# HuiyangYu/TGSFilter

Measured on NVIDIA B200. Metric: filtered Gbases/s, higher is better.
Workload: dtype u8/u64

## Files before the change

include/tgsf.h:

```cpp
#ifndef TGSF_H_
#define TGSF_H_

#include <stddef.h>
#include <stdint.h>

#ifdef __cplusplus
extern "C" {
#endif

#define TGSF_OK 0
#define TGSF_ERR_INVALID 1
#define TGSF_ERR_CUDA 2
#define TGSF_ERR_NOMEM 3
#define TGSF_ERR_STATE 4
#define TGSF_ERR_CAPACITY 5

#define TGSF_DROPINFO_N 17
#define TGSF_QUAL_HIST_N 256
#define TGSF_MAX_ADAPTERS 65536
#define TGSF_MAX_ADAPTER_LEN 2048
#define TGSF_LIB_ADAPTERS 22

#define TGSF_FLAG_FILTER 1u
#define TGSF_FLAG_ONLY_QC 2u
#define TGSF_FLAG_DISCARD_MID 4u
#define TGSF_FLAG_GZ_BLOCKS 8u
#define TGSF_FLAG_GZ_FASTA 16u

typedef struct tgsf_params {
    int32_t min_len;
    int32_t max_len;
    float min_q;
    float max_q;
    int32_t bc_len;
    int32_t head_trim;
    int32_t tail_trim;
    int32_t end_len;
    int32_t end_match_len;
    int32_t mid_match_len;
    int32_t extra_len;
    float end_sim;
    float mid_sim;
    int32_t kmer;
    int32_t min_repeat;
    int32_t qtype;
    uint32_t flags;
    int32_t n_adapters;
    const uint8_t *const *adapter_seq;
    const int32_t *adapter_len;
    int32_t max_read_len;
    int32_t n_slots;
} tgsf_params;

typedef struct tgsf_read_result {
    uint64_t sum_q;
    int32_t status;
    int32_t n_mid;
    int32_t n_5p;
    int32_t n_3p;
    int32_t piece_begin;
    int32_t n_pieces;
} tgsf_read_result;

#define TGSF_READ_EVALUATED 0
#define TGSF_READ_LOWQ 1
#define TGSF_READ_EMPTY 2

typedef struct tgsf_piece {
    uint64_t sum_q;
    int32_t read;
    int32_t start;
    int32_t len;
    int32_t repeat_len;
    int32_t status;
    int32_t contam_hits;
} tgsf_piece;

#define TGSF_PIECE_EMIT 0
#define TGSF_PIECE_SHORT_REPEAT 1
#define TGSF_PIECE_LOWQ 2
#define TGSF_PIECE_QC_ONLY 3
#define TGSF_PIECE_CONTAM 4

typedef struct tgsf_counter_layout {
    uint32_t n_u64;
    uint32_t bc_len;
    uint32_t max_bins;
    uint32_t drop_info;
    uint32_t raw_hist;
    uint32_t clean_hist;
    uint32_t raw5p_cnt;
    uint32_t raw5p_qual;
    uint32_t raw3p_cnt;
    uint32_t raw3p_qual;
    uint32_t clean5p_cnt;
    uint32_t clean5p_qual;
    uint32_t clean3p_cnt;
    uint32_t clean3p_qual;
    uint32_t raw_bin_cnt;
    uint32_t raw_bin_qual;
    uint32_t clean_bin_cnt;
    uint32_t clean_bin_qual;
} tgsf_counter_layout;

typedef struct tgsf_ctx tgsf_ctx;

const char *tgsf_version(void);
const char *tgsf_last_error(void);

int tgsf_create(int device, const tgsf_params *params, tgsf_ctx **out);
int tgsf_destroy(tgsf_ctx *ctx);

int tgsf_device_count(int *count);

int tgsf_host_alloc(void **ptr, size_t bytes);
int tgsf_host_free(void *ptr);

int tgsf_submit(tgsf_ctx *ctx, const uint8_t *bases, const uint8_t *quals, const uint64_t *offsets,
                uint32_t n_reads);
int tgsf_submit_packed(tgsf_ctx *ctx, const uint8_t *packed_bases, const uint8_t *quals, const uint64_t *offsets,
                       uint32_t n_reads, const uint64_t *exc_pos, const uint8_t *exc_byte, uint64_t n_exc);
int tgsf_pack_bases(const uint8_t *bases, uint64_t n, uint8_t *packed, uint64_t *exc_pos, uint8_t *exc_byte,
                    uint64_t exc_cap, uint64_t *n_exc);
int tgsf_submit_device(tgsf_ctx *ctx, const uint8_t *d_bases, const uint8_t *d_quals,
                       const uint64_t *d_offsets, uint32_t n_reads, uint64_t n_bases);
typedef struct tgsf_gz_span {
    uint64_t offset;
    uint32_t bytes;
    uint32_t reserved;
} tgsf_gz_span;
int tgsf_collect_gz(tgsf_ctx *ctx, uint8_t *blob, uint64_t blob_cap, uint64_t *blob_bytes, tgsf_gz_span *spans,
                    uint32_t spans_cap, uint32_t *n_spans);
int tgsf_collect(tgsf_ctx *ctx, tgsf_read_result *reads, uint32_t n_reads, tgsf_piece *pieces,
                 uint32_t pieces_cap, uint32_t *n_pieces);
int tgsf_set_contaminants(tgsf_ctx *ctx, const uint8_t *seq, const uint64_t *offsets, uint32_t n_seqs, int32_t k,
                          float min_frac, uint64_t *n_kmers);

int tgsf_last_timing(tgsf_ctx *ctx, float *kernel_ms, float *total_ms);

#define TGSF_N_STAGES 7
#define TGSF_STAGE_RAW_SCAN 0
#define TGSF_STAGE_RAW_FINAL 1
#define TGSF_STAGE_MID_SCAN 2
#define TGSF_STAGE_RESOLVE 3
#define TGSF_STAGE_REGIONS 4
#define TGSF_STAGE_KMER 5
#define TGSF_STAGE_CLEAN 6
int tgsf_last_stage_ms(tgsf_ctx *ctx, float *out, int n);

int tgsf_last_span(tgsf_ctx *ctx, float *start_ms, float *end_ms);

int tgsf_counter_layout_get(const tgsf_ctx *ctx, tgsf_counter_layout *out);
int tgsf_counters(tgsf_ctx *ctx, uint64_t *out, uint32_t n_u64);
int tgsf_counters_reset(tgsf_ctx *ctx);
int tgsf_counters_device(tgsf_ctx *ctx, void **d_ptr, uint32_t *n_u64);
int tgsf_allreduce(tgsf_ctx **ctxs, int n);
uint64_t tgsf_launch_count(const tgsf_ctx *ctx);
int tgsf_launch_shape(const tgsf_ctx *ctx, int32_t *sm_count, int32_t *last_chunk_shift);

int tgsf_prepass(int device, const uint8_t *ends5p, const uint8_t *ends3p, uint32_t n,
                 uint32_t row_len, const uint8_t *const *lib_seq, const int32_t *lib_len,
                 int32_t n_lib, float min_sim, int32_t *bases_num5p, int32_t *bases_num3p,
                 int64_t *map5p, int64_t *map3p);

typedef struct tgsf_align_result {
    int32_t edit_distance;
    int32_t n_locations;
    int32_t align_len;
    int32_t first_start, first_end, last_start, last_end;
    uint32_t loc_hash;
} tgsf_align_result;
int tgsf_align_hw(int device, const uint8_t *queries, const uint32_t *q_off, const uint8_t *targets,
                  const uint32_t *t_off, const int32_t *k, uint32_t n, tgsf_align_result *out);

#ifdef __cplusplus
}
#endif
#endif
```

tgsfilter_b200/_capi.py:

```python
from __future__ import annotations

import ctypes as C
import os

_HERE = os.path.dirname(os.path.abspath(__file__))
LIB_PATH = os.environ.get("TGSF_LIB_PATH") or os.path.join(_HERE, "libtgsf_cuda.so")

TGSF_OK = 0
TGSF_ERR_INVALID = 1
TGSF_ERR_CUDA = 2
TGSF_ERR_NOMEM = 3
TGSF_ERR_STATE = 4
TGSF_ERR_CAPACITY = 5

FLAG_FILTER = 1
FLAG_ONLY_QC = 2
FLAG_DISCARD_MID = 4
FLAG_GZ_BLOCKS = 8
FLAG_GZ_FASTA = 16

READ_EVALUATED, READ_LOWQ, READ_EMPTY = 0, 1, 2
PIECE_EMIT, PIECE_SHORT_REPEAT, PIECE_LOWQ, PIECE_QC_ONLY, PIECE_CONTAM = 0, 1, 2, 3, 4

N_STAGES = 7
STAGE_NAMES = ("raw_scan", "raw_final", "mid_scan", "resolve", "regions", "kmer", "clean")
DROPINFO_N = 17
QUAL_HIST_N = 256


class Params(C.Structure):

    _fields_ = [
        ("min_len", C.c_int32),
        ("max_len", C.c_int32),
        ("min_q", C.c_float),
        ("max_q", C.c_float),
        ("bc_len", C.c_int32),
        ("head_trim", C.c_int32),
        ("tail_trim", C.c_int32),
        ("end_len", C.c_int32),
        ("end_match_len", C.c_int32),
        ("mid_match_len", C.c_int32),
        ("extra_len", C.c_int32),
        ("end_sim", C.c_float),
        ("mid_sim", C.c_float),
        ("kmer", C.c_int32),
        ("min_repeat", C.c_int32),
        ("qtype", C.c_int32),
        ("flags", C.c_uint32),
        ("n_adapters", C.c_int32),
        ("adapter_seq", C.POINTER(C.c_char_p)),
        ("adapter_len", C.POINTER(C.c_int32)),
        ("max_read_len", C.c_int32),
        ("n_slots", C.c_int32),
    ]


class ReadResult(C.Structure):
    _fields_ = [
        ("sum_q", C.c_uint64),
        ("status", C.c_int32),
        ("n_mid", C.c_int32),
        ("n_5p", C.c_int32),
        ("n_3p", C.c_int32),
        ("piece_begin", C.c_int32),
        ("n_pieces", C.c_int32),
    ]


class Piece(C.Structure):
    _fields_ = [
        ("sum_q", C.c_uint64),
        ("read", C.c_int32),
        ("start", C.c_int32),
        ("len", C.c_int32),
        ("repeat_len", C.c_int32),
        ("status", C.c_int32),
        ("contam_hits", C.c_int32),
    ]


class CounterLayout(C.Structure):
    _fields_ = [(n, C.c_uint32) for n in (
        "n_u64", "bc_len", "max_bins", "drop_info", "raw_hist", "clean_hist",
        "raw5p_cnt", "raw5p_qual", "raw3p_cnt", "raw3p_qual",
        "clean5p_cnt", "clean5p_qual", "clean3p_cnt", "clean3p_qual",
        "raw_bin_cnt", "raw_bin_qual", "clean_bin_cnt", "clean_bin_qual")]


class AlignResult(C.Structure):
    _fields_ = [(n, C.c_int32) for n in (
        "edit_distance", "n_locations", "align_len",
        "first_start", "first_end", "last_start", "last_end")] + [("loc_hash", C.c_uint32)]


READ_RESULT_DTYPE = [("sum_q", "<u8"), ("status", "<i4"), ("n_mid", "<i4"), ("n_5p", "<i4"),
                     ("n_3p", "<i4"), ("piece_begin", "<i4"), ("n_pieces", "<i4")]
PIECE_DTYPE = [("sum_q", "<u8"), ("read", "<i4"), ("start", "<i4"), ("len", "<i4"),
               ("repeat_len", "<i4"), ("status", "<i4"), ("contam_hits", "<i4")]
ALIGN_RESULT_DTYPE = [("edit_distance", "<i4"), ("n_locations", "<i4"), ("align_len", "<i4"),
                      ("first_start", "<i4"), ("first_end", "<i4"), ("last_start", "<i4"),
                      ("last_end", "<i4"), ("loc_hash", "<u4")]

EXPORTED_SYMBOLS = (
    "tgsf_version", "tgsf_last_error", "tgsf_create", "tgsf_destroy", "tgsf_device_count", "tgsf_host_alloc",
    "tgsf_host_free", "tgsf_submit", "tgsf_submit_packed", "tgsf_pack_bases", "tgsf_submit_device", "tgsf_collect", "tgsf_collect_gz", "tgsf_last_timing", "tgsf_last_span", "tgsf_last_stage_ms",
    "tgsf_counter_layout_get", "tgsf_counters", "tgsf_counters_reset", "tgsf_counters_device",
    "tgsf_launch_count", "tgsf_launch_shape", "tgsf_allreduce", "tgsf_prepass", "tgsf_align_hw", "tgsf_set_contaminants",
)

_lib = None


def load() -> C.CDLL:
    global _lib
    if _lib is not None:
        return _lib
    if not os.path.exists(LIB_PATH):
        raise RuntimeError(
            f"{LIB_PATH} is missing: build it with __graft_entry__.build() "
            "(nvcc, sm_100a). tgsfilter_b200 has no CPU fallback.")
    lib = C.CDLL(LIB_PATH)
    vp, u8p, u64p = C.c_void_p, C.c_void_p, C.c_void_p
    lib.tgsf_version.restype = C.c_char_p
    lib.tgsf_version.argtypes = []
    lib.tgsf_last_error.restype = C.c_char_p
    lib.tgsf_last_error.argtypes = []
    lib.tgsf_create.argtypes = [C.c_int, C.POINTER(Params), C.POINTER(vp)]
    lib.tgsf_destroy.argtypes = [vp]
    lib.tgsf_device_count.argtypes = [C.POINTER(C.c_int)]
    lib.tgsf_host_alloc.argtypes = [C.POINTER(vp), C.c_size_t]
    lib.tgsf_host_free.argtypes = [vp]
    lib.tgsf_submit.argtypes = [vp, u8p, u8p, u64p, C.c_uint32]
    lib.tgsf_submit_packed.argtypes = [vp, u8p, u8p, u64p, C.c_uint32, u64p, u8p, C.c_uint64]
    lib.tgsf_pack_bases.argtypes = [u8p, C.c_uint64, u8p, u64p, u8p, C.c_uint64, C.POINTER(C.c_uint64)]
    lib.tgsf_submit_device.argtypes = [vp, u8p, u8p, u64p, C.c_uint32, C.c_uint64]
    lib.tgsf_collect.argtypes = [vp, vp, C.c_uint32, vp, C.c_uint32, C.POINTER(C.c_uint32)]
    lib.tgsf_collect_gz.argtypes = [vp, vp, C.c_uint64, C.POINTER(C.c_uint64), vp, C.c_uint32, C.POINTER(C.c_uint32)]
    lib.tgsf_last_timing.argtypes = [vp, C.POINTER(C.c_float), C.POINTER(C.c_float)]
    lib.tgsf_last_span.argtypes = [vp, C.POINTER(C.c_float), C.POINTER(C.c_float)]
    lib.tgsf_last_stage_ms.argtypes = [vp, C.POINTER(C.c_float), C.c_int]
    lib.tgsf_counter_layout_get.argtypes = [vp, C.POINTER(CounterLayout)]
    lib.tgsf_counters.argtypes = [vp, u64p, C.c_uint32]
    lib.tgsf_counters_reset.argtypes = [vp]
    lib.tgsf_counters_device.argtypes = [vp, C.POINTER(vp), C.POINTER(C.c_uint32)]
    lib.tgsf_launch_count.restype = C.c_uint64
    lib.tgsf_launch_count.argtypes = [vp]
    lib.tgsf_launch_shape.argtypes = [vp, C.POINTER(C.c_int32), C.POINTER(C.c_int32)]
    lib.tgsf_allreduce.argtypes = [C.POINTER(vp), C.c_int]
    lib.tgsf_prepass.argtypes = [C.c_int, u8p, u8p, C.c_uint32, C.c_uint32,
                                 C.POINTER(C.c_char_p), C.POINTER(C.c_int32), C.c_int32, C.c_float,
                                 vp, vp, vp, vp]
    lib.tgsf_align_hw.argtypes = [C.c_int, u8p, vp, u8p, vp, vp, C.c_uint32, vp]
    lib.tgsf_set_contaminants.argtypes = [vp, u8p, u64p, C.c_uint32, C.c_int32, C.c_float, C.POINTER(C.c_uint64)]
    for name in EXPORTED_SYMBOLS:
        fn = getattr(lib, name)
        if fn.restype is C.c_int and name not in ("tgsf_version", "tgsf_last_error",
                                                   "tgsf_launch_count"):
            fn.restype = C.c_int
    _lib = lib
    return lib


class TgsfError(RuntimeError):
    def __init__(self, code: int, where: str):
        msg = ""
        try:
            msg = load().tgsf_last_error().decode("utf-8", "replace")
        except Exception:
            pass
        super().__init__(f"{where} failed with status {code}: {msg}")
        self.code = code


def check(code: int, where: str) -> None:
    if code != TGSF_OK:
        raise TgsfError(code, where)
```

tgsfilter_b200/csrc/adapters.cuh:

```cuda
#pragma once
#include "common.cuh"
#include "myers.cuh"

#define MID_THREADS 128
#define RES_THREADS 128

struct AdapterCtx {
    const DevAdapter *ad;
    const u64 *peq_pool;
};

static __device__ __forceinline__ AdapterTables adapter_tables(const AdapterCtx &C, int a) {
    const DevAdapter A = C.ad[a];
    AdapterTables T;
    T.hw = C.peq_pool + A.peq_off;
    T.fw = T.hw + 256 * A.nw;
    T.rv = T.fw + 256 * A.nw;
    T.qlen = A.qlen;
    return T;
}

struct MidScanArgs {
    int a[2];
    int end_len;
    int chunk_shift;
    u32 chunk_stride;
    int n_adapters;
};

template <int NW>
static __device__ void mid_chunk_record(const u64 *__restrict__ tab, int tab_stride, int qlen,
                                        const uint8_t *__restrict__ bases, u64 sb, u64 ob, u64 oe,
                                        int d, u32 &cnt, u64 &first) {
    Myers<NW> s;
    myers_init_hw<NW>(s, qlen);
    cnt = 0;
    first = 0;
    for (u64 p = sb; p < oe; ++p) {
        myers_step<NW, 0, true>(s, tab + (u32)bases[p] * tab_stride, 0);
        if (p >= ob && s.score == d) {
            if (cnt == 0) first = p;
            ++cnt;
        }
    }
}

template <int NW>
static __device__ __noinline__ int mid_replay_group(const u64 *P0, const u64 *M0, u32 w0, u32 w1,
                                                    const u64 *tab, int tab_stride, int best) {
    u64 tP[NW], tM[NW];
#pragma unroll
    for (int w = 0; w < NW; ++w) { tP[w] = P0[w]; tM[w] = M0[w]; }
    const u32 wd[2] = {w0, w1};
#pragma unroll 1
    for (int j = 0; j < 8; ++j) {
        const u32 byte = (wd[j >> 2] >> (8 * (j & 3))) & 0xffu;
        myers_step_state<NW>(tP, tM, tab + byte * tab_stride);
        best = min(best, myers_score<NW>(tP, tM));
    }
    return best;
}

template <int NW, int AP>
__global__ void __launch_bounds__(MID_THREADS, (NW * AP <= 2) ? 6 : 3)
k_mid_scan_dyn(DevBatch B, AdapterCtx C, MidScanArgs M, const ChunkEntry *__restrict__ chunks,
               const u32 *__restrict__ perm, const u32 *__restrict__ n_chunks_ptr,
               uint8_t *__restrict__ chunk_min,
               u32 *__restrict__ chunk_cnt, u64 *__restrict__ chunk_first,
               u32 *__restrict__ best_mid, u32 *__restrict__ work_ctr) {
    const u32 n_chunks = *n_chunks_ptr;
    extern __shared__ __align__(16) u64 s_peq_smem[];
    DevAdapter A[AP];
#pragma unroll
    for (int x = 0; x < AP; ++x) A[x] = C.ad[M.a[x]];
    const u64 *s_peq = s_peq_smem;
    if (NW > 4) {
        s_peq = C.peq_pool + A[0].peq_off;
    } else {
#pragma unroll
        for (int x = 0; x < AP; ++x) {
            const u64 *src = C.peq_pool + A[x].peq_off;
            for (int i = threadIdx.x; i < 256 * NW; i += MID_THREADS)
                s_peq_smem[(i / NW) * (AP * NW) + x * NW + (i % NW)] = src[i];
        }
        __syncthreads();
    }
    constexpr int TS = AP * NW;
    const u64 chunk_len = 1ull << M.chunk_shift;
    int halo = 0, qmin = 0x7fffffff;
#pragma unroll
    for (int x = 0; x < AP; ++x) {
        halo = max(halo, A[x].halo_mid);
        qmin = min(qmin, A[x].qlen);
    }
    const uint4 *__restrict__ b16 = (const uint4 *)B.bases;

    const u32 lane = threadIdx.x & 31u;
    for (;;) {
        u32 it = 0;
        if (lane == 0) it = atomicAdd(work_ctr, 32u);
        it = __shfl_sync(0xffffffffu, it, 0);
        if (it >= n_chunks) break;
        it += lane;
        if (it >= n_chunks) continue;
        const u32 ci = perm[it];
        const ChunkEntry ce = chunks[ci];
        const u64 rs = B.offsets[ce.read];
        const u64 re = B.offsets[ce.read + 1];
        const i64 tsm = (i64)(re - rs) - 2 * (i64)M.end_len;
        const u64 mb = rs + (u64)M.end_len, me = re - (u64)M.end_len;
        const u64 cb = (u64)ce.chunk << M.chunk_shift;
        const u64 ob = max(cb, mb), oe = min(cb + chunk_len, me);
        u64 sb = ob > (u64)halo ? ob - (u64)halo : 0;
        if (sb < mb) sb = mb;

        u64 Pv[AP][NW], Mv[AP][NW];
        int score[AP], best[AP];
        bool on[AP];
#pragma unroll
        for (int x = 0; x < AP; ++x) {
            Myers<NW> s0;
            myers_init_hw<NW>(s0, A[x].qlen);
#pragma unroll
            for (int w = 0; w < NW; ++w) { Pv[x][w] = s0.Pv[w]; Mv[x][w] = s0.Mv[w]; }
            score[x] = A[x].qlen;
            best[x] = 0x7fffffff;
            on[x] = A[x].k_mid > 0 && tsm >= (i64)A[x].qlen;
        }
        if (tsm >= (i64)qmin) {
            u64 p = sb;
            while (p < oe && (p & 15ull)) {
                const u64 *eq = s_peq + (u32)B.bases[p] * TS;
#pragma unroll
                for (int x = 0; x < AP; ++x) {
                    myers_step_state<NW>(Pv[x], Mv[x], eq + x * NW);
                    score[x] = myers_score<NW>(Pv[x], Mv[x]);
                    if (p >= ob) best[x] = min(best[x], score[x]);
                }
                ++p;
            }
            for (; p + 16 <= oe; p += 16) {
                const uint4 v = __ldg(b16 + (p >> 4));
                const u32 wd[4] = {v.x, v.y, v.z, v.w};
                const bool tracked = p >= ob;
#pragma unroll
                for (int h = 0; h < 2; ++h) {
                    u64 Pv0[AP][NW], Mv0[AP][NW];
#pragma unroll
                    for (int x = 0; x < AP; ++x)
#pragma unroll
                        for (int w = 0; w < NW; ++w) { Pv0[x][w] = Pv[x][w]; Mv0[x][w] = Mv[x][w]; }
#pragma unroll
                    for (int j = 8 * h; j < 8 * h + 8; ++j) {
                        const u32 byte = (wd[j >> 2] >> (8 * (j & 3))) & 0xffu;
                        const u64 *eq = s_peq + byte * TS;
#pragma unroll
                        for (int x = 0; x < AP; ++x) myers_step_state<NW>(Pv[x], Mv[x], eq + x * NW);
                    }
                    if (tracked) {
#pragma unroll
                        for (int x = 0; x < AP; ++x) {
                            const int s_end = myers_score<NW>(Pv[x], Mv[x]);
                            if (((score[x] + s_end - 8 + 1) >> 1) <= min(A[x].k_mid, best[x] - 1))
                                best[x] = mid_replay_group<NW>(Pv0[x], Mv0[x], wd[2 * h], wd[2 * h + 1],
                                                               s_peq + x * NW, TS, best[x]);
                            score[x] = s_end;
                        }
                    }
                }
                if (!tracked && p + 16 >= ob) {
#pragma unroll
                    for (int x = 0; x < AP; ++x) score[x] = myers_score<NW>(Pv[x], Mv[x]);
                }
            }
            for (; p < oe; ++p) {
                const u64 *eq = s_peq + (u32)B.bases[p] * TS;
#pragma unroll
                for (int x = 0; x < AP; ++x) {
                    myers_step_state<NW>(Pv[x], Mv[x], eq + x * NW);
                    score[x] = myers_score<NW>(Pv[x], Mv[x]);
                    if (p >= ob) best[x] = min(best[x], score[x]);
                }
            }
        }
#pragma unroll
        for (int x = 0; x < AP; ++x) {
            uint8_t result = 255;
            const u64 slot = (u64)M.a[x] * M.chunk_stride + ci;
            if (on[x] && best[x] <= A[x].k_mid) {
                result = (uint8_t)min(best[x], 254);
                atomicMin(best_mid + (u64)ce.read * M.n_adapters + M.a[x], (u32)best[x]);
                u32 cnt;
                u64 first;
                mid_chunk_record<NW>(s_peq + x * NW, TS, A[x].qlen, B.bases, sb, ob, oe, best[x], cnt, first);
                chunk_cnt[slot] = cnt;
                chunk_first[slot] = first | ((u64)best[x] << 48);
            }
            chunk_min[slot] = result;
        }
    }
}

template <int NW, typename F>
static __device__ void mid_for_each_end(const DevBatch &B, const AdapterTables &T,
                                        const DevAdapter &A, int a, int end_len, int chunk_shift,
                                        u32 r, int d, const u32 *__restrict__ chunk_off,
                                        const ChunkEntry *__restrict__ chunks, u32 chunk_stride,
                                        const uint8_t *__restrict__ chunk_min,
                                        const u32 *__restrict__ chunk_hits,
                                        const u64 *__restrict__ chunk_first, F f) {
    const u64 rs = B.offsets[r], re = B.offsets[r + 1];
    const u64 mb = rs + (u64)end_len, me = re - (u64)end_len;
    for (u32 ci = chunk_off[r]; ci < chunk_off[r + 1]; ++ci) {
        const u64 slot = (u64)a * chunk_stride + ci;
        if (chunk_min[slot] != (uint8_t)min(d, 254)) continue;
        const u64 rec = chunk_first[slot];
        if ((int)(rec >> 48) != d) continue;
        const u64 first = rec & ((1ull << 48) - 1);
        u32 left = chunk_hits[slot];
        const u64 cb = (u64)chunks[ci].chunk << chunk_shift;
        const u64 oe = min(cb + (1ull << chunk_shift), me);
        u64 sb = first > (u64)A.halo_mid ? first - (u64)A.halo_mid : 0;
        if (sb < mb) sb = mb;
        Myers<NW> s;
        myers_init_hw<NW>(s, T.qlen);
        for (u64 p = sb; p < oe && left; ++p) {
            myers_step<NW, 0, true>(s, T.hw + (u32)__ldg(B.bases + p) * NW, 0);
            if (p >= first && s.score == d) {
                --left;
                if (!f(p)) return;
            }
        }
    }
}

template <int NW>
__global__ void __launch_bounds__(RES_THREADS)
k_mid_count(DevBatch B, AdapterCtx C, int a, int end_len, int n_adapters,
            const u32 *__restrict__ best_mid, const u32 *__restrict__ chunk_off, u32 chunk_stride,
            const uint8_t *__restrict__ chunk_min, const u32 *__restrict__ chunk_cnt,
            const u64 *__restrict__ chunk_first, u32 *__restrict__ mid_n, u64 *scratch,
            u64 scratch_stride) {
    const DevAdapter A = C.ad[a];
    const AdapterTables T = adapter_tables(C, a);
    const u64 tid = (u64)blockIdx.x * RES_THREADS + threadIdx.x;
    for (u32 r = (u32)tid; r < B.n_reads; r += gridDim.x * RES_THREADS) {
        const u32 bd = best_mid[(u64)r * n_adapters + a];
        if (bd == 0xffffffffu) continue;
        const int d = (int)bd;
        const uint8_t tag = (uint8_t)min(d, 254);
        u32 count = 0;
        u64 first = 0;
        for (u32 ci = chunk_off[r]; ci < chunk_off[r + 1]; ++ci) {
            const u64 slot = (u64)a * chunk_stride + ci;
            if (chunk_min[slot] != tag) continue;
            const u64 rec = chunk_first[slot];
            if ((int)(rec >> 48) != d) continue;
            if (count == 0) first = rec & ((1ull << 48) - 1);
            count += chunk_cnt[slot];
        }
        const u64 mb = B.offsets[r] + (u64)end_len;
        const u64 s0 = shw_start<NW>(T, B.bases, mb, first, d);
        int ok = mlen_decision(T.qlen, (int)(first - s0 + 1), d, A.thr_mid);
        if (ok < 0) {
            const int alen = nw_alignment_len<NW>(T, B.bases, s0, first, d, scratch + tid, scratch_stride);
            ok = (alen - d >= A.thr_mid) ? 1 : 0;
        }
        mid_n[(u64)r * n_adapters + a] = ok ? count : 0u;
    }
}

template <int NW>
__global__ void __launch_bounds__(RES_THREADS)
k_mid_emit(DevBatch B, AdapterCtx C, int a, int end_len, int chunk_shift, int extra_len,
           int n_adapters, const u32 *__restrict__ best_mid, const u32 *__restrict__ chunk_off,
           const ChunkEntry *__restrict__ chunks, u32 chunk_stride,
           const uint8_t *__restrict__ chunk_min, const u32 *__restrict__ chunk_hits,
           const u64 *__restrict__ chunk_first, const u32 *__restrict__ mid_n,
           const u32 *__restrict__ mid_off, Region *__restrict__ pool,
           const u32 *__restrict__ dev_status) {
    if (*dev_status != DEV_STATUS_OK) return;
    const DevAdapter A = C.ad[a];
    const AdapterTables T = adapter_tables(C, a);
    for (u32 r = blockIdx.x * RES_THREADS + threadIdx.x; r < B.n_reads;
         r += gridDim.x * RES_THREADS) {
        const u64 key = (u64)r * n_adapters + a;
        const u32 n = mid_n[key];
        if (n == 0) continue;
        const int d = (int)best_mid[key];
        const u64 rs = B.offsets[r];
        const int tLen = (int)(B.offsets[r + 1] - rs);
        const u64 mb = rs + (u64)end_len;
        Region *out = pool + mid_off[key];
        u32 i = 0;
        mid_for_each_end<NW>(B, T, A, a, end_len, chunk_shift, r, d, chunk_off, chunks, chunk_stride,
                             chunk_min, chunk_hits, chunk_first, [&](u64 p) {
                                 const u64 s0 = shw_start<NW>(T, B.bases, mb, p, d);
                                 int ts = (int)(s0 - rs) - extra_len;
                                 int te = (int)(p - rs) + 1 + extra_len;
                                 if (ts < 0) ts = 0;
                                 if (te > tLen) te = tLen;
                                 out[i].s = ts;
                                 out[i].e = te;
                                 ++i;
                                 return i < n;
                             });
    }
}

template <int NW, int AP>
__global__ void __launch_bounds__(RES_THREADS)
k_ends(DevBatch B, AdapterCtx C, int a0, int a1, int end_len, int n_adapters,
       const int *__restrict__ read_active, int *__restrict__ end_n, int *__restrict__ end_pos,
       u64 *scratch, u64 scratch_stride) {
    extern __shared__ u64 s_tab_smem[];
    const int aidx[2] = {a0, a1};
    DevAdapter A[AP];
    AdapterTables T[AP];
    const u64 *rvhw[AP];
#pragma unroll
    for (int x = 0; x < AP; ++x) {
        A[x] = C.ad[aidx[x]];
        const u64 *tab = C.peq_pool + A[x].peq_off;
        if (NW <= 4) {
            u64 *dst = s_tab_smem + (size_t)x * 4 * 256 * NW;
            for (int i = threadIdx.x; i < 4 * 256 * NW; i += RES_THREADS) dst[i] = tab[i];
            tab = dst;
        }
        T[x].hw = tab;
        T[x].fw = tab + 256 * NW;
        T[x].rv = tab + 512 * NW;
        T[x].qlen = A[x].qlen;
        rvhw[x] = tab + 768 * NW;
    }
    if (NW <= 4) __syncthreads();
    const u64 tid = (u64)blockIdx.x * RES_THREADS + threadIdx.x;
    const u64 total = (u64)B.n_reads * 2;
    for (u64 w = tid; w < total; w += (u64)gridDim.x * RES_THREADS) {
        const int side = w >= B.n_reads ? 1 : 0;
        const u32 r = (u32)(side ? w - B.n_reads : w);
        const bool active = read_active[r] != 0;
        const u64 rs = B.offsets[r];
        const int tLen = (int)(B.offsets[r + 1] - rs);
        u64 lo[AP], hi[AP];
        Myers<NW> s[AP];
        int d[AP], cnt[AP];
        u64 first[AP], last[AP];
        u64 lo_min = ~0ull, hi_max = 0;
#pragma unroll
        for (int x = 0; x < AP; ++x) {
            int checkLen = end_len + A[x].end_extra;
            if (checkLen > tLen) checkLen = tLen;
            const bool on = active && A[x].k_end > 0 && checkLen >= 5;
            lo[x] = side == 0 ? rs : rs + (u64)(tLen - checkLen);
            hi[x] = on ? lo[x] + (u64)checkLen : lo[x];
            if (on) { lo_min = min(lo_min, lo[x]); hi_max = max(hi_max, hi[x]); }
            myers_init_hw<NW>(s[x], T[x].qlen);
            d[x] = 0x7fffffff;
            cnt[x] = 0;
            first[x] = last[x] = 0;
        }
#pragma unroll 4
        for (u64 p = lo_min; p < hi_max; ++p) {
            const u32 byte = (u32)__ldg(B.bases + p);
#pragma unroll
            for (int x = 0; x < AP; ++x) {
                if (AP == 1 || (p >= lo[x] && p < hi[x])) {
                    myers_step<NW, 0, true>(s[x], T[x].hw + byte * NW, 0);
                    if (s[x].score < d[x]) { d[x] = s[x].score; cnt[x] = 1; first[x] = p; last[x] = p; }
                    else if (s[x].score == d[x]) { ++cnt[x]; last[x] = p; }
                }
            }
        }
#pragma unroll
        for (int x = 0; x < AP; ++x) {
            if (AP == 2 && x == 1 && a1 == a0) break;
            const u64 oidx = ((u64)r * n_adapters + aidx[x]) * 2 + side;
            int n_loc = 0, pos = 0;
            if (hi[x] > lo[x] && d[x] <= A[x].k_end) {
                const u64 s0 = shw_start<NW>(T[x], B.bases, lo[x], first[x], d[x]);
                int ok = mlen_decision(T[x].qlen, (int)(first[x] - s0 + 1), d[x], A[x].thr_end);
                if (ok < 0) {
                    const int alen = nw_alignment_len<NW>(T[x], B.bases, s0, first[x], d[x], scratch + tid, scratch_stride);
                    ok = (alen - d[x] >= A[x].thr_end) ? 1 : 0;
                }
                if (ok) {
                    n_loc = cnt[x];
                    if (side == 0) {
                        pos = (int)(last[x] - rs) + 1;
                    } else {
                        Myers<NW> sr;
                        myers_init_hw<NW>(sr, T[x].qlen);
                        u64 leftmost = s0;
#pragma unroll 4
                        for (u64 p = hi[x]; p-- > lo[x];) {
                            myers_step<NW, 0, true>(sr, rvhw[x] + (u32)__ldg(B.bases + p) * NW, 0);
                            if (sr.score == d[x]) leftmost = p;
                        }
                        pos = (int)(leftmost - rs);
                    }
                }
            }
            end_n[oidx] = n_loc;
            end_pos[oidx] = pos;
        }
    }
}
```

tgsfilter_b200/csrc/common.cuh:

```cuda
#pragma once
#include <cuda_runtime.h>
#include <stdint.h>

#include "../../include/tgsf.h"
#include "../../include/tgsf_layout.h"

typedef unsigned long long u64;
typedef long long i64;
typedef unsigned int u32;

#define TGSF_SM_COUNT_FALLBACK 148

#define SCAN_BIN 100
#define SCAN_TILE_BINS 32
#define SCAN_TILE (SCAN_BIN * SCAN_TILE_BINS)
#define MID_CHUNK_SHIFT_MIN 10
#define MID_CHUNK_SHIFT_MAX 12

struct DevAdapter {
    int qlen;
    int nw;
    int k_mid;
    int k_end;
    int thr_mid;
    int thr_end;
    int end_extra;
    int halo_mid;
    u32 peq_off;
};

struct DevParams {
    int min_len, max_len;
    double min_q, max_q;
    int bc_len, head_trim, tail_trim, end_len, extra_len;
    int kmer, min_repeat, qtype;
    u32 flags;
    int n_adapters;
    int has_qual;
    tgsf_counter_layout L;
};

struct DevBatch {
    const uint8_t *bases;
    const uint8_t *quals;
    const u64 *offsets;
    u32 n_reads;
};

struct __align__(16) TileEntry {
    u64 start;
    u32 seg;
    u32 tile;
};
#define TILE_N_BITS 12

struct __align__(8) ChunkEntry {
    u32 read;
    u32 chunk;
};

struct __align__(8) Region {
    int s, e;
};

struct __align__(16) TmpPiece {
    int read, idx, start, len;
};

#define DEV_STATUS_OK 0u
#define DEV_STATUS_POOL_OVERFLOW 1u
#define DEV_STATUS_BIN_OVERFLOW 2u

static __device__ __forceinline__ void atomic_add_u64(u64 *p, u64 v) { atomicAdd(p, v); }

static __device__ __forceinline__ u32 warp_sum_u32(u32 v) {
#pragma unroll
    for (int o = 16; o > 0; o >>= 1) v += __shfl_xor_sync(0xffffffffu, v, o);
    return v;
}
static __device__ __forceinline__ i64 warp_sum_i64(i64 v) {
#pragma unroll
    for (int o = 16; o > 0; o >>= 1) v += __shfl_xor_sync(0xffffffffu, v, o);
    return v;
}
```

tgsfilter_b200/csrc/tgsf_cuda.cu:

```cuda
#include <cuda_runtime.h>

#include <algorithm>
#include <cstdarg>
#include <cstdio>
#include <cstdlib>
#include <cstring>
#include <new>
#include <string>
#include <vector>

#include "adapters.cuh"
#include "common.cuh"
#include "contam.cuh"
#include "kmer.cuh"
#include "kmer16.cuh"
#include "gzenc.cuh"
#include "prepass.cuh"
#include "regions.cuh"
#include "scan.cuh"
#include "util.cuh"

namespace {

thread_local char g_err[512] = "";

void set_err(const char *fmt, ...) {
    va_list ap;
    va_start(ap, fmt);
    vsnprintf(g_err, sizeof(g_err), fmt, ap);
    va_end(ap);
}

#define CU(call)                                                                          \
    do {                                                                                  \
        cudaError_t e_ = (call);                                                          \
        if (e_ != cudaSuccess) {                                                          \
            set_err("%s:%d %s: %s", __FILE__, __LINE__, #call, cudaGetErrorString(e_));   \
            return TGSF_ERR_CUDA;                                                         \
        }                                                                                 \
    } while (0)

#define TRY(call)              \
    do {                       \
        int rc_ = (call);      \
        if (rc_ != TGSF_OK) return rc_; \
    } while (0)

struct DBuf {
    void *p = nullptr;
    size_t cap = 0;
    int ensure(size_t bytes) {
        if (bytes <= cap) return TGSF_OK;
        if (p) cudaFree(p);
        p = nullptr;
        cap = 0;
        size_t want = bytes + bytes / 8 + 256;
        cudaError_t e = cudaMalloc(&p, want);
        if (e != cudaSuccess) {
            set_err("cudaMalloc(%zu): %s", want, cudaGetErrorString(e));
            return TGSF_ERR_NOMEM;
        }
        cap = want;
        return TGSF_OK;
    }
    void release() {
        if (p) cudaFree(p);
        p = nullptr;
        cap = 0;
    }
    template <typename T> T *as() const { return (T *)p; }
};

struct HBuf {
    void *p = nullptr;
    size_t cap = 0;
    int ensure(size_t bytes) {
        if (bytes <= cap) return TGSF_OK;
        if (p) cudaFreeHost(p);
        p = nullptr;
        cap = 0;
        size_t want = bytes + bytes / 8 + 256;
        cudaError_t e = cudaHostAlloc(&p, want, cudaHostAllocDefault);
        if (e != cudaSuccess) {
            set_err("cudaHostAlloc(%zu): %s", want, cudaGetErrorString(e));
            return TGSF_ERR_NOMEM;
        }
        cap = want;
        return TGSF_OK;
    }
    void release() {
        if (p) cudaFreeHost(p);
        p = nullptr;
        cap = 0;
    }
};

inline int round_nw(int nw);

struct AdapterSet {
    std::vector<DevAdapter> host;
    DBuf d_ad, d_peq;
    int max_q = 0, min_q = 0x7fffffff, max_nw = 1;
    int max_cols = 0;

    int build(const uint8_t *const *seq, const int32_t *len, int n) {
        host.resize((size_t)n);
        size_t words = 0;
        for (int a = 0; a < n; ++a) {
            DevAdapter &A = host[(size_t)a];
            memset(&A, 0, sizeof(A));
            A.qlen = len[a];
            A.nw = round_nw((len[a] + 63) / 64);
            A.peq_off = (u32)words;
            words += (size_t)4 * 256 * (size_t)std::max(A.nw, 1);
            if (A.qlen > 0) {
                max_q = std::max(max_q, A.qlen);
                min_q = std::min(min_q, A.qlen);
                max_nw = std::max(max_nw, A.nw);
            }
        }
        std::vector<u64> peq(words, 0);
        for (int a = 0; a < n; ++a) {
            const DevAdapter &A = host[(size_t)a];
            const int q = A.qlen, nw = A.nw;
            if (q <= 0) continue;
            const int W = 64 * nw - q;
            u64 *hw = peq.data() + A.peq_off, *fw = hw + 256 * nw, *rv = fw + 256 * nw, *rvhw = rv + 256 * nw;
            for (int b = 0; b < 256; ++b)
                for (int i = 0; i < W; ++i) {
                    hw[b * nw + (i >> 6)] |= 1ull << (i & 63);
                    rvhw[b * nw + (i >> 6)] |= 1ull << (i & 63);
                }
            for (int i = 0; i < q; ++i) {
                const int b = seq[a][i];
                hw[b * nw + ((W + i) >> 6)] |= 1ull << ((W + i) & 63);
                fw[b * nw + (i >> 6)] |= 1ull << (i & 63);
                const int br = seq[a][q - 1 - i];
                rv[br * nw + (i >> 6)] |= 1ull << (i & 63);
                rvhw[br * nw + ((W + i) >> 6)] |= 1ull << ((W + i) & 63);
            }
        }
        TRY(d_peq.ensure(std::max<size_t>(words, 1) * sizeof(u64)));
        if (words) {
            cudaError_t e = cudaMemcpy(d_peq.p, peq.data(), words * sizeof(u64), cudaMemcpyHostToDevice);
            if (e != cudaSuccess) { set_err("peq upload: %s", cudaGetErrorString(e)); return TGSF_ERR_CUDA; }
        }
        return TGSF_OK;
    }
    int upload() {
        max_cols = 16;
        for (auto &A : host) max_cols = std::max(max_cols, 2 * A.qlen + 2);
        TRY(d_ad.ensure(std::max<size_t>(host.size(), 1) * sizeof(DevAdapter)));
        if (!host.empty()) {
            cudaError_t e = cudaMemcpy(d_ad.p, host.data(), host.size() * sizeof(DevAdapter), cudaMemcpyHostToDevice);
            if (e != cudaSuccess) { set_err("adapter upload: %s", cudaGetErrorString(e)); return TGSF_ERR_CUDA; }
        }
        return TGSF_OK;
    }
    AdapterCtx ctx() const {
        AdapterCtx c;
        c.ad = d_ad.as<DevAdapter>();
        c.peq_pool = d_peq.as<u64>();
        return c;
    }
    void release() { d_ad.release(); d_peq.release(); }
};

#define TGSF_SCRATCH_BUDGET (2ull << 30)
struct Scratch {
    DBuf buf;
    static size_t per_thread(int cols, int nw) { return (size_t)cols * (size_t)(2 * nw + 1) * sizeof(u64); }
    static int grid_for(int default_grid, int threads_per_cta, int cols, int nw) {
        const u64 fit = TGSF_SCRATCH_BUDGET / ((u64)per_thread(cols, nw) * (u64)threads_per_cta);
        return (int)std::max<u64>(1, std::min<u64>((u64)default_grid, fit));
    }
    template <typename ADS>
    int ensure(const ADS &ads, int default_grid, int threads_per_cta) {
        size_t need = 0;
        for (const auto &A : ads) {
            if (A.qlen <= 0 || A.nw <= 0) continue;
            const int cols = 2 * A.qlen + 2;
            need = std::max(need, (size_t)grid_for(default_grid, threads_per_cta, cols, A.nw) * threads_per_cta * per_thread(cols, A.nw));
        }
        return buf.ensure(std::max<size_t>(need, 256));
    }
};

struct DevHeader {
    u32 status;
    u32 tmp_cursor;
    u32 sort_cursor;
    u32 gz_overflow;
    unsigned long long gz_cursor;
    u32 kmer_work;
    u32 kmer_long;
};

struct Slot {
    cudaStream_t stream = nullptr;
    cudaStream_t stream2 = nullptr;
    cudaEvent_t ev_fork = nullptr, ev_join = nullptr;
    cudaEvent_t ev_start = nullptr, ev_k0 = nullptr, ev_k1 = nullptr, ev_end = nullptr;
    cudaEvent_t ev_stage[TGSF_N_STAGES + 1] = {};
    bool busy = false;
    DBuf in_bases, in_quals, in_offsets, in_packed, in_exc_pos, in_exc_val;
    DevBatch B{};
    u64 n_bases = 0;
    bool has_qual = false;
    DBuf seg_start, seg_len, seg_sum, seg_flag, tile_cnt, tile_off, tiles;
    DBuf read_active, piece_cnt, piece_begin, chunk_cnt, chunk_off, chunks, chunk_min, chunk_hits, chunk_first, chunk_perm, chunk_hist;
    int chunk_shift = MID_CHUNK_SHIFT_MIN;
    DBuf best_mid, mid_n, mid_off, end_n, end_pos, pool, sortbuf, tmp, pieces, res, header;
    DBuf scan_tmp, kmer_long_list, mid_work, gz_blob, gz_spans;
    DBuf contam_cnt, contam_off, contam_chunks;
    Scratch scratch, scratch2;
    u32 pool_cap = 0, pieces_cap = 0, chunks_cap = 0, tiles_cap = 0;
    HBuf h_res, h_pieces, h_header;
    u32 h_pieces_copied = 0;
    float kernel_ms = 0, total_ms = 0;
};

struct ContamSet {
    DBuf table, pf_bits;
    u64 mask = 0;
    u64 n_keys = 0;
    u64 ppm = 0;
    int k = 0;
    bool installed() const { return table.p != nullptr; }
    void release() { table.release(); pf_bits.release(); n_keys = 0; }
};

}

struct tgsf_ctx {
    int device = 0;
    int sm_count = TGSF_SM_COUNT_FALLBACK;
    DevParams P{};
    AdapterSet ads;
    ContamSet contam;
    DBuf counters;
    std::vector<Slot> slots;
    u32 head = 0, tail = 0, outstanding = 0;
    u64 launches = 0;
    int kmer16_ctas_per_sm = 2;
    int mid_ctas_per_sm = 0;
    int res_ctas_per_sm = 6;
    bool fork_ends = true;
    u32 kmer16_list_cap = KMER16_LIST_CAP;
    float last_kernel_ms = 0, last_total_ms = 0;
    float last_stage_ms[TGSF_N_STAGES] = {};
    int last_chunk_shift = 0;
    cudaEvent_t ev_epoch = nullptr;
    float last_span_start = 0, last_span_end = 0;
};

namespace {

inline u32 cdiv(u64 a, u64 b) { return (u32)((a + b - 1) / b); }

int exclusive_scan(tgsf_ctx *c, cudaStream_t st, const u32 *in, u32 *out, u32 n, u32 *tmp, size_t tmp_words) {
    if (n == 0) {
        CU(cudaMemsetAsync(out, 0, sizeof(u32), st));
        return TGSF_OK;
    }
    const u32 nb = cdiv(n, SCANB_TILE);
    if ((size_t)nb * 2 + 8 > tmp_words) { set_err("scan scratch too small"); return TGSF_ERR_INVALID; }
    u32 *sums = tmp;
    u32 *sums_sc = tmp + nb;
    u32 *rest = tmp + 2 * (size_t)nb + 1;
    k_scan_block<<<nb, UTIL_THREADS, 0, st>>>(in, out, n, sums);
    c->launches++;
    if (nb == 1) {
        CU(cudaMemcpyAsync(out + n, sums, sizeof(u32), cudaMemcpyDeviceToDevice, st));
        return TGSF_OK;
    }
    TRY(exclusive_scan(c, st, sums, sums_sc, nb, rest, tmp_words - (2 * (size_t)nb + 1)));
    k_scan_add<<<cdiv(n, UTIL_THREADS), UTIL_THREADS, 0, st>>>(out, n, sums_sc, sums_sc + nb);
    c->launches++;
    return TGSF_OK;
}

int slot_init(Slot &s) {
    CU(cudaStreamCreateWithFlags(&s.stream, cudaStreamNonBlocking));
    CU(cudaStreamCreateWithFlags(&s.stream2, cudaStreamNonBlocking));
    CU(cudaEventCreateWithFlags(&s.ev_fork, cudaEventDisableTiming));
    CU(cudaEventCreateWithFlags(&s.ev_join, cudaEventDisableTiming));
    CU(cudaEventCreate(&s.ev_start));
    CU(cudaEventCreate(&s.ev_k0));
    CU(cudaEventCreate(&s.ev_k1));
    CU(cudaEventCreate(&s.ev_end));
    for (auto &e : s.ev_stage) CU(cudaEventCreate(&e));
    return TGSF_OK;
}

void slot_release(Slot &s) {
    DBuf *bufs[] = {&s.in_bases, &s.in_quals, &s.in_offsets, &s.in_packed, &s.in_exc_pos, &s.in_exc_val, &s.seg_start, &s.seg_len, &s.seg_sum,
                    &s.seg_flag, &s.tile_cnt, &s.tile_off, &s.tiles, &s.read_active, &s.piece_cnt,
                    &s.piece_begin, &s.chunk_cnt, &s.chunk_off, &s.chunks, &s.chunk_min, &s.chunk_hits, &s.chunk_first, &s.chunk_perm, &s.chunk_hist,
                    &s.best_mid, &s.mid_n, &s.mid_off, &s.end_n, &s.end_pos, &s.pool, &s.sortbuf,
                    &s.tmp, &s.pieces, &s.res, &s.header, &s.scan_tmp, &s.kmer_long_list, &s.mid_work, &s.gz_blob, &s.gz_spans, &s.scratch.buf, &s.scratch2.buf,
                    &s.contam_cnt, &s.contam_off, &s.contam_chunks};
    for (DBuf *b : bufs) b->release();
    s.h_res.release();
    s.h_pieces.release();
    s.h_header.release();
    if (s.ev_start) cudaEventDestroy(s.ev_start);
    if (s.ev_k0) cudaEventDestroy(s.ev_k0);
    if (s.ev_k1) cudaEventDestroy(s.ev_k1);
    if (s.ev_end) cudaEventDestroy(s.ev_end);
    for (auto &e : s.ev_stage)
        if (e) cudaEventDestroy(e);
    if (s.ev_fork) cudaEventDestroy(s.ev_fork);
    if (s.ev_join) cudaEventDestroy(s.ev_join);
    if (s.stream2) cudaStreamDestroy(s.stream2);
    if (s.stream) cudaStreamDestroy(s.stream);
}

int slot_reserve(tgsf_ctx *c, Slot &s, u32 n, u64 n_bases) {
    const int A = std::max(c->P.n_adapters, 1);
    if (s.pool_cap == 0) s.pool_cap = 65536;
    s.pieces_cap = n + s.pool_cap;
    s.chunk_shift = MID_CHUNK_SHIFT_MIN;
    while (s.chunk_shift < MID_CHUNK_SHIFT_MAX &&
           (n_bases >> (s.chunk_shift + 1)) >= (u64)c->sm_count * 2048ull * 4ull)
        s.chunk_shift++;
    s.chunks_cap = (u32)((n_bases >> s.chunk_shift) + 2ull * n + 16);
    s.tiles_cap = (u32)(n_bases / SCAN_TILE + (u64)s.pieces_cap + 16);
    const size_t nseg = std::max<size_t>(n, s.pieces_cap) + 1;
    TRY(s.seg_start.ensure(nseg * sizeof(u64)));
    TRY(s.seg_len.ensure(nseg * sizeof(int)));
    TRY(s.seg_sum.ensure(nseg * sizeof(u64)));
    TRY(s.seg_flag.ensure(nseg * sizeof(int)));
    TRY(s.tile_cnt.ensure(nseg * sizeof(u32)));
    TRY(s.tile_off.ensure((nseg + 1) * sizeof(u32)));
    TRY(s.tiles.ensure((size_t)s.tiles_cap * sizeof(TileEntry)));
    TRY(s.read_active.ensure(((size_t)n + 1) * sizeof(int)));
    TRY(s.piece_cnt.ensure(((size_t)n + 1) * sizeof(u32)));
    TRY(s.piece_begin.ensure(((size_t)n + 2) * sizeof(u32)));
    TRY(s.chunk_cnt.ensure(((size_t)n + 1) * sizeof(u32)));
    TRY(s.chunk_off.ensure(((size_t)n + 2) * sizeof(u32)));
    TRY(s.chunks.ensure((size_t)s.chunks_cap * sizeof(ChunkEntry)));
    TRY(s.chunk_min.ensure((size_t)s.chunks_cap * (size_t)A));
    TRY(s.chunk_hits.ensure((size_t)s.chunks_cap * (size_t)A * sizeof(u32)));
    TRY(s.chunk_first.ensure((size_t)s.chunks_cap * (size_t)A * sizeof(u64)));
    TRY(s.chunk_perm.ensure((size_t)s.chunks_cap * sizeof(u32)));
    TRY(s.chunk_hist.ensure(CHUNK_BUCKETS * sizeof(u32)));
    TRY(s.best_mid.ensure(((size_t)n * A + 1) * sizeof(u32)));
    TRY(s.mid_n.ensure(((size_t)n * A + 1) * sizeof(u32)));
    TRY(s.mid_off.ensure(((size_t)n * A + 2) * sizeof(u32)));
    TRY(s.end_n.ensure(((size_t)n * A * 2 + 1) * sizeof(int)));
    TRY(s.end_pos.ensure(((size_t)n * A * 2 + 1) * sizeof(int)));
    TRY(s.pool.ensure((size_t)s.pool_cap * sizeof(Region)));
    TRY(s.sortbuf.ensure((size_t)s.pool_cap * 5 * sizeof(Region)));
    TRY(s.tmp.ensure((size_t)s.pieces_cap * sizeof(TmpPiece)));
    TRY(s.pieces.ensure((size_t)s.pieces_cap * sizeof(tgsf_piece)));
    TRY(s.res.ensure(((size_t)n + 1) * sizeof(tgsf_read_result)));
    TRY(s.header.ensure(sizeof(DevHeader)));
    TRY(s.mid_work.ensure((size_t)A * sizeof(u32)));
    if (c->P.flags & TGSF_FLAG_GZ_BLOCKS) {
        const u64 syms = n_bases * ((c->P.flags & TGSF_FLAG_GZ_FASTA) ? 1ull : 2ull);
        TRY(s.gz_blob.ensure((size_t)(syms + syms / 8 + (u64)s.pieces_cap * 512ull + 4096ull)));
        TRY(s.gz_spans.ensure((size_t)s.pieces_cap * sizeof(GzSpan)));
    }
    const size_t scan_words = 4 * (std::max<size_t>(nseg, (size_t)n * A) / SCANB_TILE) + 4096;
    TRY(s.scan_tmp.ensure(scan_words * sizeof(u32)));
    TRY(s.h_res.ensure(((size_t)n + 1) * sizeof(tgsf_read_result)));
    TRY(s.h_pieces.ensure(((size_t)n + 4096) * sizeof(tgsf_piece)));
    TRY(s.h_header.ensure(sizeof(DevHeader)));
    TRY(s.scratch.ensure(c->ads.host, c->sm_count * c->res_ctas_per_sm, RES_THREADS));
    if (c->fork_ends) TRY(s.scratch2.ensure(c->ads.host, c->sm_count * c->res_ctas_per_sm, RES_THREADS));
    return TGSF_OK;
}

inline int round_nw(int nw) { return nw <= 4 ? nw : nw <= 8 ? 8 : nw <= 16 ? 16 : 32; }

template <typename F>
int for_nw(int nw, F f) {
    switch (nw) {
        case 1: return f(std::integral_constant<int, 1>());
        case 2: return f(std::integral_constant<int, 2>());
        case 3: return f(std::integral_constant<int, 3>());
        case 4: return f(std::integral_constant<int, 4>());
        case 8: return f(std::integral_constant<int, 8>());
        case 16: return f(std::integral_constant<int, 16>());
        case 32: return f(std::integral_constant<int, 32>());
        default: set_err("adapter longer than %d", TGSF_MAX_ADAPTER_LEN); return TGSF_ERR_INVALID;
    }
}

int check_launch(const char *what) {
    cudaError_t e = cudaGetLastError();
    if (e != cudaSuccess) {
        set_err("launch %s: %s", what, cudaGetErrorString(e));
        return TGSF_ERR_CUDA;
    }
    return TGSF_OK;
}

int launch_scan_pass(tgsf_ctx *c, Slot &s, u32 n_seg, u64 *bin_cnt, u64 *bin_qual) {
    cudaStream_t st = s.stream;
    const size_t scan_words = s.scan_tmp.cap / sizeof(u32);
    TRY(exclusive_scan(c, st, s.tile_cnt.as<u32>(), s.tile_off.as<u32>(), n_seg, s.scan_tmp.as<u32>(), scan_words));
    if (n_seg) {
        k_fill_tiles<<<cdiv(n_seg, 256), 256, 0, st>>>(s.tile_off.as<u32>(), n_seg, s.seg_start.as<u64>(), s.seg_len.as<int>(), s.tiles.as<TileEntry>());
        c->launches++;
    }
    const int grid = c->sm_count;
    u32 *status = &s.header.as<DevHeader>()->status;
    auto launch = [&](auto kern, size_t smem) {
        kern<<<grid, SCAN_THREADS, smem, st>>>(s.B.bases, s.B.quals, s.tiles.as<TileEntry>(), s.tile_off.as<u32>() + n_seg,
                                               s.seg_sum.as<u64>(), bin_cnt, bin_qual, c->P.qtype, c->P.L.max_bins, status);
    };
    if (!s.has_qual) launch(k_scan_tiles_dyn<false, false>, SCAN_SMEM_BYTES);
    else if (scan_needs_wide(s.tiles_cap, grid, c->P.qtype)) launch(k_scan_tiles_dyn<true, true>, SCAN_SMEM_BYTES_WIDE);
    else launch(k_scan_tiles_dyn<true, false>, SCAN_SMEM_BYTES);
    c->launches++;
    return check_launch("k_scan_tiles");
}

int launch_ends_qc(tgsf_ctx *c, Slot &s, u32 n_seg, const int *flag, bool clean) {
    if (c->P.bc_len <= 0 || n_seg == 0) return TGSF_OK;
    u64 *C = c->counters.as<u64>();
    const tgsf_counter_layout &L = c->P.L;
    u64 *cnt5 = C + (clean ? L.clean5p_cnt : L.raw5p_cnt), *q5 = C + (clean ? L.clean5p_qual : L.raw5p_qual);
    u64 *cnt3 = C + (clean ? L.clean3p_cnt : L.raw3p_cnt), *q3 = C + (clean ? L.clean3p_qual : L.raw3p_qual);
    const int grid = std::min<u32>((u32)c->sm_count * 4, cdiv(n_seg, ENDS_THREADS / 32));
    const size_t sm = c->P.bc_len <= ENDS_SMEM_ROWS ? (size_t)2 * c->P.bc_len * 10 * sizeof(u32) : 0;
    if (s.has_qual)
        k_ends_qc<true><<<grid, ENDS_THREADS, sm, s.stream>>>(s.B.bases, s.B.quals, n_seg, s.seg_start.as<u64>(),
                                                              s.seg_len.as<int>(), flag, c->P.bc_len, c->P.qtype,
                                                              cnt5, q5, cnt3, q3);
    else
        k_ends_qc<false><<<grid, ENDS_THREADS, sm, s.stream>>>(s.B.bases, s.B.quals, n_seg, s.seg_start.as<u64>(),
                                                               s.seg_len.as<int>(), flag, c->P.bc_len, c->P.qtype,
                                                               cnt5, q5, cnt3, q3);
    c->launches++;
    return check_launch("k_ends_qc");
}

int launch_head(tgsf_ctx *c, Slot &s) {
    cudaStream_t st = s.stream;
    const u32 n = s.B.n_reads;
    const int A = c->P.n_adapters;
    u64 *C = c->counters.as<u64>();
    const tgsf_counter_layout &L = c->P.L;
    DevParams P = c->P;
    P.has_qual = s.has_qual;
    CU(cudaMemsetAsync(s.header.p, 0, sizeof(DevHeader), st));
    u32 *status = &s.header.as<DevHeader>()->status;
    if (n == 0) {
        for (int i = 0; i <= 4; ++i) CU(cudaEventRecord(s.ev_stage[i], st));
        return TGSF_OK;
    }

    CU(cudaEventRecord(s.ev_stage[0], st));
    k_read_segments<<<cdiv(n, 256), 256, 0, st>>>(s.B, s.seg_start.as<u64>(), s.seg_len.as<int>(),
                                                  s.seg_sum.as<u64>(), s.tile_cnt.as<u32>(), L.max_bins, status);
    c->launches++;
    TRY(launch_scan_pass(c, s, n, C + L.raw_bin_cnt, C + L.raw_bin_qual));
    CU(cudaEventRecord(s.ev_stage[1], st));
    if (s.has_qual)
        k_finalize_raw<true><<<cdiv(n, REG_THREADS), REG_THREADS, 0, st>>>(
            s.B, P, s.seg_sum.as<u64>(), s.res.as<tgsf_read_result>(), s.read_active.as<int>(),
            s.piece_cnt.as<u32>(), C);
    else
        k_finalize_raw<false><<<cdiv(n, REG_THREADS), REG_THREADS, 0, st>>>(
            s.B, P, s.seg_sum.as<u64>(), s.res.as<tgsf_read_result>(), s.read_active.as<int>(),
            s.piece_cnt.as<u32>(), C);
    c->launches++;
    TRY(launch_ends_qc(c, s, n, nullptr, false));
    CU(cudaEventRecord(s.ev_stage[2], st));

    const bool filter = (P.flags & TGSF_FLAG_FILTER) != 0;
    if (filter && A > 0) {
        const AdapterCtx ACe = c->ads.ctx();
        const int res_grid_e = c->sm_count * c->res_ctas_per_sm;
        auto launch_ends = [&](cudaStream_t es, Scratch &sc) -> int {
            const AdapterCtx &AC = ACe;
            const int res_grid = res_grid_e;
        for (int nw : {1, 2, 3, 4, 8, 16, 32}) {
            std::vector<int> grp;
            for (int a = 0; a < A; ++a)
                if (c->ads.host[(size_t)a].nw == nw) grp.push_back(a);
            const size_t step = nw <= 2 ? 2 : 1;
            for (size_t i = 0; i < grp.size(); i += step) {
                const int a0 = grp[i], a1 = (step == 2 && i + 1 < grp.size()) ? grp[i + 1] : grp[i];
                const int qmax = std::max(c->ads.host[(size_t)a0].qlen, c->ads.host[(size_t)a1].qlen);
                const int grid_a = Scratch::grid_for(res_grid, RES_THREADS, 2 * qmax + 2, nw);
                const u64 stride_a = (u64)grid_a * RES_THREADS;
                TRY(for_nw(nw, [&](auto nwc) {
                    constexpr int NW = decltype(nwc)::value;
                    if constexpr (NW <= 2) {
                        if (a1 != a0)
                            k_ends<NW, 2><<<grid_a, RES_THREADS, 2 * 4 * 256 * NW * sizeof(u64), es>>>(
                                s.B, AC, a0, a1, P.end_len, A, s.read_active.as<int>(), s.end_n.as<int>(), s.end_pos.as<int>(),
                                sc.buf.as<u64>(), stride_a);
                        else
                            k_ends<NW, 1><<<grid_a, RES_THREADS, 4 * 256 * NW * sizeof(u64), es>>>(
                                s.B, AC, a0, a0, P.end_len, A, s.read_active.as<int>(), s.end_n.as<int>(), s.end_pos.as<int>(),
                                sc.buf.as<u64>(), stride_a);
                    } else {
                        k_ends<NW, 1><<<grid_a, RES_THREADS, NW <= 4 ? 4 * 256 * NW * sizeof(u64) : 0, es>>>(
                            s.B, AC, a0, a0, P.end_len, A, s.read_active.as<int>(), s.end_n.as<int>(), s.end_pos.as<int>(),
                            sc.buf.as<u64>(), stride_a);
                    }
                    c->launches++;
                    return check_launch("k_ends");
                }));
            }
        }
            return TGSF_OK;
        };
        if (c->fork_ends) {
            CU(cudaEventRecord(s.ev_fork, st));
            CU(cudaStreamWaitEvent(s.stream2, s.ev_fork, 0));
            TRY(launch_ends(s.stream2, s.scratch2));
            CU(cudaEventRecord(s.ev_join, s.stream2));
        }
        k_count_chunks<<<cdiv(n, 256), 256, 0, st>>>(s.B, s.read_active.as<int>(), P.end_len, s.chunk_shift, c->ads.min_q,
                                                     s.chunk_cnt.as<u32>(), s.best_mid.as<u32>(),
                                                     s.mid_n.as<u32>(), A);
        c->launches++;
        TRY(exclusive_scan(c, st, s.chunk_cnt.as<u32>(), s.chunk_off.as<u32>(), n, s.scan_tmp.as<u32>(),
                           s.scan_tmp.cap / sizeof(u32)));
        k_fill_chunks<<<cdiv(n, 256), 256, 0, st>>>(s.B, s.chunk_off.as<u32>(), P.end_len, s.chunk_shift, s.chunks.as<ChunkEntry>());
        c->launches++;
        CU(cudaMemsetAsync(s.chunk_hist.p, 0, CHUNK_BUCKETS * sizeof(u32), st));
        k_chunk_hist<<<cdiv(n, UTIL_THREADS), UTIL_THREADS, 0, st>>>(s.B, s.chunk_off.as<u32>(), s.chunks.as<ChunkEntry>(),
                                                                   P.end_len, s.chunk_shift, s.chunk_hist.as<u32>());
        k_chunk_base<<<1, 32, 0, st>>>(s.chunk_hist.as<u32>());
        k_chunk_scatter<<<cdiv(n, UTIL_THREADS), UTIL_THREADS, 0, st>>>(s.B, s.chunk_off.as<u32>(), s.chunks.as<ChunkEntry>(),
                                                                      P.end_len, s.chunk_shift, s.chunk_hist.as<u32>(),
                                                                      s.chunk_perm.as<u32>());
        c->launches += 3;
        const AdapterCtx AC = c->ads.ctx();
        const u32 *n_chunks_ptr = s.chunk_off.as<u32>() + n;
        const int res_grid = c->sm_count * c->res_ctas_per_sm;
        int mid_launch = 0;
        CU(cudaMemsetAsync(s.mid_work.p, 0, (size_t)A * sizeof(u32), st));
        for (int nw : {1, 2, 3, 4, 8, 16, 32}) {
            std::vector<int> grp;
            for (int a = 0; a < A; ++a)
                if (c->ads.host[(size_t)a].nw == nw && c->ads.host[(size_t)a].k_mid > 0) grp.push_back(a);
            const size_t step = nw <= 4 ? 2 : 1;
            for (size_t i = 0; i < grp.size(); i += step) {
                const bool pair = step == 2 && i + 1 < grp.size();
                MidScanArgs M;
                M.a[0] = grp[i];
                M.a[1] = pair ? grp[i + 1] : grp[i];
                M.end_len = P.end_len;
                M.chunk_shift = s.chunk_shift;
                M.chunk_stride = s.chunks_cap;
                M.n_adapters = A;
                TRY(for_nw(nw, [&](auto nwc) {
                    constexpr int NW = decltype(nwc)::value;
                    auto launch = [&](auto kern, size_t smem) {
                        int occ = 0;
                        if (cudaOccupancyMaxActiveBlocksPerMultiprocessor(&occ, kern, MID_THREADS, smem) != cudaSuccess || occ < 1) occ = 4;
                        if (c->mid_ctas_per_sm > 0) occ = std::min(occ, c->mid_ctas_per_sm);
                        kern<<<c->sm_count * occ, MID_THREADS, smem, st>>>(
                            s.B, AC, M, s.chunks.as<ChunkEntry>(), s.chunk_perm.as<u32>(), n_chunks_ptr,
                            s.chunk_min.as<uint8_t>(), s.chunk_hits.as<u32>(), s.chunk_first.as<u64>(),
                            s.best_mid.as<u32>(), s.mid_work.as<u32>() + mid_launch);
                    };
                    if constexpr (NW <= 4) {
                        if (pair) launch(k_mid_scan_dyn<NW, 2>, 256 * 2 * NW * sizeof(u64));
                        else launch(k_mid_scan_dyn<NW, 1>, 256 * NW * sizeof(u64));
                    } else {
                        launch(k_mid_scan_dyn<NW, 1>, 0);
                    }
                    c->launches++;
                    ++mid_launch;
                    return check_launch("k_mid_scan");
                }));
            }
        }
        CU(cudaEventRecord(s.ev_stage[3], st));
        for (int a = 0; a < A; ++a) {
            const DevAdapter &Ah = c->ads.host[(size_t)a];
            if (Ah.k_mid <= 0) continue;
            const int grid_a = Scratch::grid_for(res_grid, RES_THREADS, 2 * Ah.qlen + 2, Ah.nw);
            TRY(for_nw(Ah.nw, [&](auto nwc) {
                constexpr int NW = decltype(nwc)::value;
                k_mid_count<NW><<<grid_a, RES_THREADS, 0, st>>>(
                    s.B, AC, a, P.end_len, A, s.best_mid.as<u32>(), s.chunk_off.as<u32>(), s.chunks_cap,
                    s.chunk_min.as<uint8_t>(), s.chunk_hits.as<u32>(), s.chunk_first.as<u64>(),
                    s.mid_n.as<u32>(), s.scratch.buf.as<u64>(), (u64)grid_a * RES_THREADS);
                c->launches++;
                return check_launch("k_mid_count");
            }));
        }
        if (c->fork_ends) CU(cudaStreamWaitEvent(st, s.ev_join, 0));
        else TRY(launch_ends(st, s.scratch));
        TRY(exclusive_scan(c, st, s.mid_n.as<u32>(), s.mid_off.as<u32>(), n * (u32)A, s.scan_tmp.as<u32>(),
                           s.scan_tmp.cap / sizeof(u32)));
        k_check_pool<<<1, 1, 0, st>>>(s.mid_off.as<u32>() + (size_t)n * A, s.pool_cap, status);
        c->launches++;
    } else {
        CU(cudaEventRecord(s.ev_stage[3], st));
    }
    CU(cudaEventRecord(s.ev_stage[4], st));
    return check_launch("head");
}

int launch_kmer(tgsf_ctx *c, Slot &s, const DevParams &P) {
    cudaStream_t st = s.stream;
    DevHeader *H = s.header.as<DevHeader>();
    u64 *C = c->counters.as<u64>();
    tgsf_piece *pieces = s.pieces.as<tgsf_piece>();
    if (P.kmer > 16) {
        k_kmer<u64><<<c->sm_count, KMER_THREADS, KMER_SMEM_BYTES, st>>>(s.B, P, pieces, &H->tmp_cursor, C, &H->status, nullptr);
        c->launches++;
        return check_launch("k_kmer");
    }
    TRY(s.kmer_long_list.ensure((size_t)s.pieces_cap * sizeof(u32)));
    u32 *long_list = s.kmer_long_list.as<u32>();
    k_kmer_tag16<<<c->sm_count * c->kmer16_ctas_per_sm, KMER16_THREADS, KMER16_SMEM_BYTES, st>>>(
        s.B, P, pieces, &H->tmp_cursor, C, &H->status, &H->kmer_work, long_list, &H->kmer_long, c->kmer16_list_cap);
    if (P.kmer <= 12)
        k_kmer_smem<<<c->sm_count, KMER_SB_THREADS, KMER_SB_SMEM_BYTES, st>>>(s.B, P, pieces, &H->kmer_long, C, &H->status,
                                                                             long_list);
    else if (P.kmer <= 15)
        k_kmer<u32><<<c->sm_count, KMER_THREADS, KMER_SMEM_BYTES, st>>>(s.B, P, pieces, &H->kmer_long, C, &H->status, long_list);
    else
        k_kmer<u64><<<c->sm_count, KMER_THREADS, KMER_SMEM_BYTES, st>>>(s.B, P, pieces, &H->kmer_long, C, &H->status, long_list);
    c->launches += 2;
    return check_launch("k_kmer");
}

int launch_contam(tgsf_ctx *c, Slot &s) {
    cudaStream_t st = s.stream;
    const ContamSet &cs = c->contam;
    DevHeader *H = s.header.as<DevHeader>();
    const u32 cap = s.pieces_cap;
    const size_t chunks_cap = (size_t)(s.n_bases / CONTAM_CHUNK) + cap + 16;
    TRY(s.contam_cnt.ensure((size_t)cap * sizeof(u32)));
    TRY(s.contam_off.ensure(((size_t)cap + 1) * sizeof(u32)));
    TRY(s.contam_chunks.ensure(chunks_cap * sizeof(ContamChunk)));
    k_contam_count<<<cdiv(cap, 256), 256, 0, st>>>(s.pieces.as<tgsf_piece>(), &H->tmp_cursor, cap, cs.k,
                                                   s.contam_cnt.as<u32>(), &H->status);
    c->launches++;
    TRY(exclusive_scan(c, st, s.contam_cnt.as<u32>(), s.contam_off.as<u32>(), cap, s.scan_tmp.as<u32>(),
                       s.scan_tmp.cap / sizeof(u32)));
    k_contam_fill<<<cdiv(cap, 256), 256, 0, st>>>(s.B, s.pieces.as<tgsf_piece>(), s.contam_off.as<u32>(), cap, cs.k,
                                                  s.contam_chunks.as<ContamChunk>());
    c->launches++;
    if (cs.pf_bits.p)
        k_contam_screen<true><<<c->sm_count, CONTAM_THREADS, CONTAM_PF_SMEM_BYTES, st>>>(
            s.B.bases, s.contam_chunks.as<ContamChunk>(), s.contam_off.as<u32>() + cap, cs.k, cs.table.as<u64>(), cs.mask,
            cs.pf_bits.as<u32>(), s.pieces.as<tgsf_piece>(), &H->status);
    else
        k_contam_screen<false><<<c->sm_count * 4, CONTAM_THREADS, 0, st>>>(
            s.B.bases, s.contam_chunks.as<ContamChunk>(), s.contam_off.as<u32>() + cap, cs.k, cs.table.as<u64>(), cs.mask,
            nullptr, s.pieces.as<tgsf_piece>(), &H->status);
    c->launches++;
    k_contam_decide<<<cdiv(cap, 256), 256, 0, st>>>(s.pieces.as<tgsf_piece>(), &H->tmp_cursor, cap, cs.k, cs.ppm,
                                                    &H->status);
    c->launches++;
    return check_launch("contam");
}

int launch_tail(tgsf_ctx *c, Slot &s) {
    cudaStream_t st = s.stream;
    const u32 n = s.B.n_reads;
    const int A = c->P.n_adapters;
    u64 *C = c->counters.as<u64>();
    const tgsf_counter_layout &L = c->P.L;
    DevParams P = c->P;
    P.has_qual = s.has_qual;
    DevHeader *H = s.header.as<DevHeader>();
    if (n == 0) {
        for (int i = 5; i <= TGSF_N_STAGES; ++i) CU(cudaEventRecord(s.ev_stage[i], st));
        return TGSF_OK;
    }
    const bool filter = (P.flags & TGSF_FLAG_FILTER) != 0;
    const AdapterCtx AC = c->ads.ctx();
    const int res_grid = c->sm_count * c->res_ctas_per_sm;
    if (filter && A > 0) {
        for (int a = 0; a < A; ++a) {
            const DevAdapter &Ah = c->ads.host[(size_t)a];
            if (Ah.k_mid <= 0) continue;
            TRY(for_nw(Ah.nw, [&](auto nwc) {
                constexpr int NW = decltype(nwc)::value;
                k_mid_emit<NW><<<res_grid, RES_THREADS, 0, st>>>(
                    s.B, AC, a, P.end_len, s.chunk_shift, P.extra_len, A, s.best_mid.as<u32>(), s.chunk_off.as<u32>(),
                    s.chunks.as<ChunkEntry>(), s.chunks_cap, s.chunk_min.as<uint8_t>(), s.chunk_hits.as<u32>(),
                    s.chunk_first.as<u64>(), s.mid_n.as<u32>(), s.mid_off.as<u32>(), s.pool.as<Region>(), &H->status);
                c->launches++;
                return check_launch("k_mid_emit");
            }));
        }
    } else if (filter) {
        CU(cudaMemsetAsync(s.mid_n.p, 0, sizeof(u32), st));
    }
    CU(cudaMemsetAsync(s.pieces.p, 0, (size_t)std::min<u32>(s.pieces_cap, n + 4096) * sizeof(tgsf_piece), st));
    k_regions<<<cdiv(n, REG_THREADS), REG_THREADS, 0, st>>>(
        s.B, P, s.read_active.as<int>(), s.end_n.as<int>(), s.end_pos.as<int>(), s.mid_n.as<u32>(),
        s.mid_off.as<u32>(), s.pool.as<Region>(), s.sortbuf.as<Region>(), s.pool_cap * 5, &H->sort_cursor,
        s.res.as<tgsf_read_result>(), s.piece_cnt.as<u32>(), s.tmp.as<TmpPiece>(), s.pieces_cap,
        &H->tmp_cursor, C, &H->status);
    c->launches++;
    TRY(exclusive_scan(c, st, s.piece_cnt.as<u32>(), s.piece_begin.as<u32>(), n, s.scan_tmp.as<u32>(),
                       s.scan_tmp.cap / sizeof(u32)));
    const u32 place_n = std::max(n, s.pieces_cap);
    k_place_pieces<<<cdiv(place_n, 256), 256, 0, st>>>(s.tmp.as<TmpPiece>(), &H->tmp_cursor,
                                                       s.piece_begin.as<u32>(), s.res.as<tgsf_read_result>(),
                                                       s.pieces.as<tgsf_piece>(), n,
                                                       (P.flags & TGSF_FLAG_ONLY_QC) ? 1 : 0, &H->status);
    c->launches++;
    CU(cudaEventRecord(s.ev_stage[5], st));
    if (!(P.flags & TGSF_FLAG_ONLY_QC)) {
        if (P.min_repeat > 0) TRY(launch_kmer(c, s, P));
        if (c->contam.installed()) TRY(launch_contam(c, s));
        CU(cudaEventRecord(s.ev_stage[6], st));
        k_piece_segments_dyn<<<cdiv(s.pieces_cap, 256), 256, 0, st>>>(
            s.B, s.pieces.as<tgsf_piece>(), &H->tmp_cursor, s.pieces_cap, s.seg_start.as<u64>(),
            s.seg_len.as<int>(), s.seg_sum.as<u64>(), s.tile_cnt.as<u32>(), &H->status);
        c->launches++;
        TRY(launch_scan_pass(c, s, s.pieces_cap, C + L.clean_bin_cnt, C + L.clean_bin_qual));
        if (s.has_qual)
            k_finalize_clean_dyn<true><<<cdiv(s.pieces_cap, REG_THREADS), REG_THREADS, 0, st>>>(
                P, s.pieces.as<tgsf_piece>(), &H->tmp_cursor, s.pieces_cap, s.seg_sum.as<u64>(),
                s.seg_flag.as<int>(), C, &H->status);
        else
            k_finalize_clean_dyn<false><<<cdiv(s.pieces_cap, REG_THREADS), REG_THREADS, 0, st>>>(
                P, s.pieces.as<tgsf_piece>(), &H->tmp_cursor, s.pieces_cap, s.seg_sum.as<u64>(),
                s.seg_flag.as<int>(), C, &H->status);
        c->launches++;
        TRY(launch_ends_qc(c, s, s.pieces_cap, s.seg_flag.as<int>(), true));
    } else {
        CU(cudaEventRecord(s.ev_stage[6], st));
    }
    if ((P.flags & TGSF_FLAG_GZ_BLOCKS) && !(P.flags & TGSF_FLAG_ONLY_QC)) {
        const bool fasta = (P.flags & TGSF_FLAG_GZ_FASTA) || !s.has_qual;
        const u64 syms = s.n_bases * (fasta ? 1ull : 2ull);
        const u64 used_cap = std::min<u64>(s.gz_blob.cap, syms + syms / 8 + (u64)s.pieces_cap * 512ull + 4096ull) & ~3ull;
        CU(cudaMemsetAsync(s.gz_blob.p, 0, (size_t)used_cap, st));
        k_gz_encode<<<c->sm_count * 6, GZ_THREADS, 0, st>>>(s.B, s.pieces.as<tgsf_piece>(), &H->tmp_cursor, fasta ? 1 : 0,
                                                          s.gz_blob.as<u32>(), used_cap, &H->gz_cursor,
                                                          s.gz_spans.as<GzSpan>(), &H->gz_overflow, &H->status);
        c->launches++;
    }
    CU(cudaEventRecord(s.ev_stage[7], st));
    return check_launch("tail");
}

int enqueue_d2h(tgsf_ctx *c, Slot &s) {
    (void)c;
    cudaStream_t st = s.stream;
    const u32 n = s.B.n_reads;
    CU(cudaMemcpyAsync(s.h_header.p, s.header.p, sizeof(DevHeader), cudaMemcpyDeviceToHost, st));
    if (n) CU(cudaMemcpyAsync(s.h_res.p, s.res.p, (size_t)n * sizeof(tgsf_read_result), cudaMemcpyDeviceToHost, st));
    s.h_pieces_copied = std::min<u32>(s.pieces_cap, n + 4096);
    if (s.h_pieces_copied)
        CU(cudaMemcpyAsync(s.h_pieces.p, s.pieces.p, (size_t)s.h_pieces_copied * sizeof(tgsf_piece),
                           cudaMemcpyDeviceToHost, st));
    return TGSF_OK;
}

int run_pipeline(tgsf_ctx *c, Slot &s) {
    TRY(launch_head(c, s));
    TRY(launch_tail(c, s));
    CU(cudaEventRecord(s.ev_k1, s.stream));
    TRY(enqueue_d2h(c, s));
    CU(cudaEventRecord(s.ev_end, s.stream));
    return TGSF_OK;
}

int validate_params(const tgsf_params *p) {
    if (!p) { set_err("params is NULL"); return TGSF_ERR_INVALID; }
    if (p->n_adapters < 0 || p->n_adapters > TGSF_MAX_ADAPTERS) { set_err("n_adapters out of range"); return TGSF_ERR_INVALID; }
    if (p->n_adapters > 0 && (!p->adapter_seq || !p->adapter_len)) { set_err("adapter arrays missing"); return TGSF_ERR_INVALID; }
    for (int a = 0; a < p->n_adapters; ++a)
        if (p->adapter_len[a] <= 0 || p->adapter_len[a] > TGSF_MAX_ADAPTER_LEN || !p->adapter_seq[a]) {
            set_err("adapter %d has invalid length %d", a, p->adapter_len[a]);
            return TGSF_ERR_INVALID;
        }
    if ((p->flags & TGSF_FLAG_FILTER) && p->n_adapters > 0 && !(p->end_sim > 0.0f && p->mid_sim > 0.0f)) {
        set_err("end_sim / mid_sim must be > 0 when filtering");
        return TGSF_ERR_INVALID;
    }
    if (p->min_repeat > 0 && (p->kmer < 1 || p->kmer > 31)) { set_err("kmer must be in [1,31]"); return TGSF_ERR_INVALID; }
    if (p->bc_len < 0 || p->end_len < 0 || p->extra_len < 0) { set_err("negative length parameter"); return TGSF_ERR_INVALID; }
    if (p->n_slots < 0 || p->n_slots > 4) { set_err("n_slots out of range"); return TGSF_ERR_INVALID; }
    return TGSF_OK;
}

void fill_thresholds(DevAdapter &A, const tgsf_params *p) {
    const int qLen = A.qlen;
    const float endSim = p->end_sim, midSim = p->mid_sim;
    auto min_mlen = [&](float sim, int match_len) {
        int m = 0;
        for (; m <= qLen; ++m) {
            float s = static_cast<float>(m) / qLen;
            if (s >= sim) break;
        }
        return std::max(m, match_len);
    };
    A.k_mid = std::min(qLen - p->mid_match_len + 1, qLen - 1);
    A.k_end = std::min(qLen - p->end_match_len + 1, qLen - 1);
    A.thr_mid = min_mlen(midSim, p->mid_match_len);
    A.thr_end = min_mlen(endSim, p->end_match_len);
    if (A.thr_mid > qLen) A.k_mid = 0;
    if (A.thr_end > qLen) A.k_end = 0;
    A.end_extra = endSim > 0.0f ? int(qLen / endSim) : 0;
    A.halo_mid = A.k_mid > 0 ? ((qLen + A.k_mid - 1 + 15) / 16) * 16 : 0;
}

}

extern "C" {

const char *tgsf_version(void) { return "libtgsf_cuda 0.1 (sm_100a; TGSFilter v1.11 per-read path)"; }
const char *tgsf_last_error(void) { return g_err; }

int tgsf_create(int device, const tgsf_params *params, tgsf_ctx **out) {
    if (!out) { set_err("out is NULL"); return TGSF_ERR_INVALID; }
    *out = nullptr;
    TRY(validate_params(params));
    CU(cudaSetDevice(device));
    tgsf_ctx *c = new (std::nothrow) tgsf_ctx();
    if (!c) return TGSF_ERR_NOMEM;
    c->device = device;
    cudaDeviceProp prop;
    CU(cudaGetDeviceProperties(&prop, device));
    c->sm_count = prop.multiProcessorCount;
    DevParams &P = c->P;
    P.min_len = params->min_len;
    P.max_len = params->max_len;
    P.min_q = (double)params->min_q;
    P.max_q = (double)params->max_q;
    P.bc_len = params->bc_len;
    P.head_trim = params->head_trim;
    P.tail_trim = params->tail_trim;
    P.end_len = params->end_len;
    P.extra_len = params->extra_len;
    P.kmer = params->kmer;
    P.min_repeat = params->min_repeat;
    P.qtype = params->qtype;
    P.flags = params->flags;
    P.n_adapters = params->n_adapters;
    P.has_qual = 1;
    tgsf_make_layout(params->bc_len, params->max_read_len, &P.L);

    int rc = c->ads.build((const uint8_t *const *)params->adapter_seq, params->adapter_len, params->n_adapters);
    if (rc == TGSF_OK) {
        for (auto &A : c->ads.host) fill_thresholds(A, params);
        rc = c->ads.upload();
    }
    if (rc == TGSF_OK) rc = c->counters.ensure((size_t)P.L.n_u64 * sizeof(u64));
    if (rc == TGSF_OK && cudaMemset(c->counters.p, 0, (size_t)P.L.n_u64 * sizeof(u64)) != cudaSuccess) rc = TGSF_ERR_CUDA;
    const int ns = params->n_slots > 0 ? params->n_slots : 2;
    c->slots.resize((size_t)ns);
    for (int i = 0; i < ns && rc == TGSF_OK; ++i) rc = slot_init(c->slots[(size_t)i]);
    if (rc == TGSF_OK && (cudaEventCreate(&c->ev_epoch) != cudaSuccess ||
                          cudaEventRecord(c->ev_epoch, c->slots[0].stream) != cudaSuccess ||
                          cudaEventSynchronize(c->ev_epoch) != cudaSuccess)) {
        set_err("epoch event: %s", cudaGetErrorString(cudaGetLastError()));
        rc = TGSF_ERR_CUDA;
    }
    if (rc == TGSF_OK) {
        cudaError_t e1 = cudaFuncSetAttribute(k_scan_tiles_dyn<true, false>, cudaFuncAttributeMaxDynamicSharedMemorySize, SCAN_SMEM_BYTES);
        cudaError_t e2 = cudaFuncSetAttribute(k_scan_tiles_dyn<false, false>, cudaFuncAttributeMaxDynamicSharedMemorySize, SCAN_SMEM_BYTES);
        if (e1 == cudaSuccess) e1 = cudaFuncSetAttribute(k_scan_tiles_dyn<true, true>, cudaFuncAttributeMaxDynamicSharedMemorySize, SCAN_SMEM_BYTES_WIDE);
        if (const char *e = getenv("TGSF_MID_CTAS")) c->mid_ctas_per_sm = atoi(e);
        if (const char *e = getenv("TGSF_FORK_ENDS")) c->fork_ends = atoi(e) != 0;
        if (const char *e = getenv("TGSF_RES_CTAS")) c->res_ctas_per_sm = std::max(1, std::min(16, atoi(e)));
        if (const char *e = getenv("TGSF_SM_COUNT")) c->sm_count = std::max(1, std::min(c->sm_count, atoi(e)));
        if (const char *e = getenv("TGSF_KMER16_LIST_CAP")) c->kmer16_list_cap = (u32)std::min<long>(std::max<long>(atol(e), 32), (long)KMER16_LIST_CAP);
        cudaError_t e3 = cudaFuncSetAttribute(k_kmer<u32>, cudaFuncAttributeMaxDynamicSharedMemorySize, KMER_SMEM_BYTES);
        cudaError_t e4 = cudaFuncSetAttribute(k_kmer<u64>, cudaFuncAttributeMaxDynamicSharedMemorySize, KMER_SMEM_BYTES);
        if (e4 == cudaSuccess) e4 = cudaFuncSetAttribute(k_kmer_smem, cudaFuncAttributeMaxDynamicSharedMemorySize, KMER_SB_SMEM_BYTES);
        if (e3 == cudaSuccess) e3 = cudaFuncSetAttribute(k_kmer_tag16, cudaFuncAttributeMaxDynamicSharedMemorySize, KMER16_SMEM_BYTES);
        if (e3 == cudaSuccess) e3 = cudaFuncSetAttribute(k_contam_screen<true>, cudaFuncAttributeMaxDynamicSharedMemorySize, CONTAM_PF_SMEM_BYTES);
        if (e3 == cudaSuccess) {
            int occ = 0;
            if (cudaOccupancyMaxActiveBlocksPerMultiprocessor(&occ, k_kmer_tag16, KMER16_THREADS, KMER16_SMEM_BYTES) == cudaSuccess && occ >= 1)
                c->kmer16_ctas_per_sm = occ;
        }
        if (e1 != cudaSuccess || e2 != cudaSuccess || e3 != cudaSuccess || e4 != cudaSuccess) {
            set_err("cudaFuncSetAttribute(smem): %s", cudaGetErrorString(e1 != cudaSuccess ? e1 : e2 != cudaSuccess ? e2 : e3 != cudaSuccess ? e3 : e4));
            rc = TGSF_ERR_CUDA;
        }
    }
    if (rc != TGSF_OK) {
        tgsf_destroy(c);
        return rc;
    }
    *out = c;
    return TGSF_OK;
}

int tgsf_destroy(tgsf_ctx *c) {
    if (!c) return TGSF_OK;
    cudaSetDevice(c->device);
    cudaDeviceSynchronize();
    for (auto &s : c->slots) slot_release(s);
    if (c->ev_epoch) cudaEventDestroy(c->ev_epoch);
    c->ads.release();
    c->contam.release();
    c->counters.release();
    delete c;
    return TGSF_OK;
}

int tgsf_set_contaminants(tgsf_ctx *c, const uint8_t *seq, const uint64_t *offsets, uint32_t n_seqs, int32_t k,
                          float min_frac, uint64_t *n_kmers) {
    if (!c || !offsets || !n_kmers || n_seqs == 0) { set_err("tgsf_set_contaminants: missing argument"); return TGSF_ERR_INVALID; }
    if (c->outstanding) { set_err("tgsf_set_contaminants with %u batch(es) outstanding", c->outstanding); return TGSF_ERR_STATE; }
    if (k < CONTAM_K_MIN || k > CONTAM_K_MAX) { set_err("contaminant k must be in [%d,%d], got %d", CONTAM_K_MIN, CONTAM_K_MAX, k); return TGSF_ERR_INVALID; }
    const double fd = (double)min_frac;
    const long long ppm = fd == fd && fd >= 0.0 && fd <= 2.0 ? llround(fd * 1e6) : -1;
    if (ppm < 1 || ppm > 1000000) { set_err("contaminant min_frac must give ppm in [1,1000000], got %g", fd); return TGSF_ERR_INVALID; }
    if (offsets[0] != 0) { set_err("contaminant offsets[0] must be 0"); return TGSF_ERR_INVALID; }
    for (uint32_t i = 0; i < n_seqs; ++i)
        if (offsets[i + 1] < offsets[i]) { set_err("contaminant offsets not ascending at %u", i); return TGSF_ERR_INVALID; }
    const u64 n_bytes = offsets[n_seqs];
    if (n_bytes < (u64)k || !seq) { set_err("contaminant set has no valid %d-mer", k); return TGSF_ERR_INVALID; }
    if (n_bytes > (1ull << 36)) { set_err("contaminant set of %llu bytes is too large", (unsigned long long)n_bytes); return TGSF_ERR_NOMEM; }
    CU(cudaSetDevice(c->device));
    u64 cap = 1024;
    while (cap < 2 * n_bytes) cap <<= 1;
    cudaStream_t st = c->slots[0].stream;
    ContamSet next;
    DBuf d_seq, d_off, d_cnt;
    auto build = [&]() -> int {
        TRY(next.table.ensure(cap * sizeof(u64)));
        TRY(d_seq.ensure(n_bytes));
        TRY(d_off.ensure(((size_t)n_seqs + 1) * sizeof(u64)));
        TRY(d_cnt.ensure(sizeof(unsigned long long)));
        CU(cudaMemsetAsync(next.table.p, 0xFF, cap * sizeof(u64), st));
        CU(cudaMemsetAsync(d_cnt.p, 0, sizeof(unsigned long long), st));
        CU(cudaMemcpyAsync(d_seq.p, seq, n_bytes, cudaMemcpyHostToDevice, st));
        CU(cudaMemcpyAsync(d_off.p, offsets, ((size_t)n_seqs + 1) * sizeof(u64), cudaMemcpyHostToDevice, st));
        const u64 threads = (n_bytes + CONTAM_BUILD_SEG - 1) / CONTAM_BUILD_SEG;
        const u32 grid = (u32)std::min<u64>((threads + 255) / 256, (u64)c->sm_count * 16);
        k_contam_build<<<grid, 256, 0, st>>>(d_seq.as<uint8_t>(), d_off.as<u64>(), n_seqs, k, next.table.as<u64>(),
                                             cap - 1, d_cnt.as<unsigned long long>());
        c->launches++;
        TRY(check_launch("k_contam_build"));
        unsigned long long n = 0;
        CU(cudaMemcpyAsync(&n, d_cnt.p, sizeof(n), cudaMemcpyDeviceToHost, st));
        CU(cudaStreamSynchronize(st));
        next.n_keys = n;
        if (n == 0) { set_err("contaminant set has no valid %d-mer", k); return TGSF_ERR_INVALID; }
        if (n <= CONTAM_PF_MAX_KEYS) {
            TRY(next.pf_bits.ensure(CONTAM_PF_SMEM_BYTES));
            CU(cudaMemsetAsync(next.pf_bits.p, 0, CONTAM_PF_SMEM_BYTES, st));
            k_contam_bitmap<<<(u32)std::min<u64>(cap / 256 + 1, (u64)c->sm_count * 8), 256, 0, st>>>(
                next.table.as<u64>(), cap, next.pf_bits.as<u32>());
            c->launches++;
            TRY(check_launch("k_contam_bitmap"));
            CU(cudaStreamSynchronize(st));
        }
        return TGSF_OK;
    };
    const int rc = build();
    d_seq.release();
    d_off.release();
    d_cnt.release();
    if (rc != TGSF_OK) {
        next.release();
        return rc;
    }
    next.mask = cap - 1;
    next.ppm = (u64)ppm;
    next.k = k;
    c->contam.release();
    c->contam = next;
    next.table.p = next.pf_bits.p = nullptr;
    *n_kmers = c->contam.n_keys;
    return TGSF_OK;
}

int tgsf_device_count(int *count) {
    if (!count) return TGSF_ERR_INVALID;
    *count = 0;
    CU(cudaGetDeviceCount(count));
    return TGSF_OK;
}

int tgsf_host_alloc(void **ptr, size_t bytes) {
    if (!ptr) return TGSF_ERR_INVALID;
    CU(cudaHostAlloc(ptr, bytes ? bytes : 1, cudaHostAllocDefault));
    return TGSF_OK;
}
int tgsf_host_free(void *ptr) {
    if (ptr) CU(cudaFreeHost(ptr));
    return TGSF_OK;
}

static int grow_counters_to(tgsf_ctx *c, u32 new_bins) {
    if (new_bins <= c->P.L.max_bins) return TGSF_OK;
    for (auto &s : c->slots)
        if (s.busy) CU(cudaStreamSynchronize(s.stream));
    const tgsf_counter_layout OL = c->P.L;
    tgsf_counter_layout NL;
    tgsf_make_layout(OL.bc_len, (int32_t)((u64)(new_bins - 1) * SCAN_BIN), &NL);
    DBuf nb;
    TRY(nb.ensure((size_t)NL.n_u64 * sizeof(u64)));
    CU(cudaMemset(nb.p, 0, (size_t)NL.n_u64 * sizeof(u64)));
    const u64 *o = c->counters.as<u64>();
    u64 *n = nb.as<u64>();
    CU(cudaMemcpy(n, o, (size_t)OL.raw_bin_cnt * sizeof(u64), cudaMemcpyDeviceToDevice));
    const u32 osec[4] = {OL.raw_bin_cnt, OL.raw_bin_qual, OL.clean_bin_cnt, OL.clean_bin_qual};
    const u32 nsec[4] = {NL.raw_bin_cnt, NL.raw_bin_qual, NL.clean_bin_cnt, NL.clean_bin_qual};
    for (int i = 0; i < 4; ++i)
        CU(cudaMemcpy(n + nsec[i], o + osec[i], (size_t)OL.max_bins * 5 * sizeof(u64), cudaMemcpyDeviceToDevice));
    c->counters.release();
    c->counters = nb;
    c->P.L = NL;
    return TGSF_OK;
}
static int grow_counters(tgsf_ctx *c, u64 longest) {
    if (longest / SCAN_BIN + 1 <= (u64)c->P.L.max_bins) return TGSF_OK;
    if (longest > 0x7fffffffull) { set_err("a read of %llu bases is longer than 2^31 - 1", (unsigned long long)longest); return TGSF_ERR_INVALID; }
    return grow_counters_to(c, (u32)(std::min<u64>(longest + longest / 4 + 1024, 0x7fffffffull) / SCAN_BIN + 1));
}

struct PackedIn {
    const uint8_t *packed = nullptr;
    const u64 *exc_pos = nullptr;
    const uint8_t *exc_val = nullptr;
    u64 n_exc = 0;
};

static int submit_common(tgsf_ctx *c, const uint8_t *bases, const uint8_t *quals, const u64 *offsets,
                         u32 n_reads, u64 n_bases, bool on_device, const PackedIn *pk = nullptr) {
    if (!c) { set_err("ctx is NULL"); return TGSF_ERR_INVALID; }
    if (n_reads && ((!bases && !pk) || !offsets)) { set_err("bases/offsets NULL"); return TGSF_ERR_INVALID; }
    if (n_reads > (1u << 24)) { set_err("more than 2^24 reads in one batch"); return TGSF_ERR_INVALID; }
    if (c->outstanding == c->slots.size()) { set_err("all %zu slots busy: collect first", c->slots.size()); return TGSF_ERR_STATE; }
    CU(cudaSetDevice(c->device));
    if (!on_device && n_reads) {
        u64 longest = 0;
        for (u32 i = 0; i < n_reads; ++i) longest = std::max<u64>(longest, offsets[i + 1] - offsets[i]);
        TRY(grow_counters(c, longest));
    }
    Slot &s = c->slots[c->head];
    s.has_qual = quals != nullptr;
    s.n_bases = n_bases;
    TRY(slot_reserve(c, s, n_reads, n_bases));
    CU(cudaEventRecord(s.ev_start, s.stream));
    if (on_device) {
        if (((uintptr_t)bases & 15) || ((uintptr_t)quals & 15)) { set_err("device streams must be 16-byte aligned"); return TGSF_ERR_INVALID; }
        s.B.bases = bases;
        s.B.quals = quals;
        s.B.offsets = offsets;
    } else {
        const size_t pad = 64;
        TRY(s.in_bases.ensure((size_t)n_bases + pad));
        TRY(s.in_offsets.ensure(((size_t)n_reads + 1) * sizeof(u64)));
        if (pk) {
            const u64 n_words = (n_bases + 15) / 16;
            TRY(s.in_bases.ensure((size_t)n_words * 16 + pad));
            TRY(s.in_packed.ensure((size_t)n_words * 4 + pad));
            if (n_bases) {
                CU(cudaMemsetAsync((uint8_t *)s.in_packed.p + (n_words - 1) * 4, 0, 4, s.stream));
                CU(cudaMemcpyAsync(s.in_packed.p, pk->packed, (size_t)((n_bases + 3) / 4), cudaMemcpyHostToDevice, s.stream));
                k_unpack_bases<<<c->sm_count * 8, 256, 0, s.stream>>>(s.in_packed.as<u32>(), n_words, s.in_bases.as<uint4>());
                c->launches++;
            }
            if (pk->n_exc) {
                TRY(s.in_exc_pos.ensure((size_t)pk->n_exc * sizeof(u64)));
                TRY(s.in_exc_val.ensure((size_t)pk->n_exc));
                CU(cudaMemcpyAsync(s.in_exc_pos.p, pk->exc_pos, (size_t)pk->n_exc * sizeof(u64), cudaMemcpyHostToDevice, s.stream));
                CU(cudaMemcpyAsync(s.in_exc_val.p, pk->exc_val, (size_t)pk->n_exc, cudaMemcpyHostToDevice, s.stream));
                k_apply_exceptions<<<c->sm_count, 256, 0, s.stream>>>(s.in_bases.as<uint8_t>(), s.in_exc_pos.as<u64>(),
                                                                     s.in_exc_val.as<uint8_t>(), pk->n_exc);
                c->launches++;
            }
        } else if (n_bases) {
            CU(cudaMemcpyAsync(s.in_bases.p, bases, (size_t)n_bases, cudaMemcpyHostToDevice, s.stream));
        }
        if (quals) {
            TRY(s.in_quals.ensure((size_t)n_bases + pad));
            if (n_bases) CU(cudaMemcpyAsync(s.in_quals.p, quals, (size_t)n_bases, cudaMemcpyHostToDevice, s.stream));
        }
        if (n_reads) CU(cudaMemcpyAsync(s.in_offsets.p, offsets, ((size_t)n_reads + 1) * sizeof(u64), cudaMemcpyHostToDevice, s.stream));
        s.B.bases = s.in_bases.as<uint8_t>();
        s.B.quals = quals ? s.in_quals.as<uint8_t>() : nullptr;
        s.B.offsets = s.in_offsets.as<u64>();
    }
    s.B.n_reads = n_reads;
    CU(cudaEventRecord(s.ev_k0, s.stream));
    TRY(run_pipeline(c, s));
    s.busy = true;
    c->head = (c->head + 1) % (u32)c->slots.size();
    c->outstanding++;
    return TGSF_OK;
}

int tgsf_submit(tgsf_ctx *c, const uint8_t *bases, const uint8_t *quals, const uint64_t *offsets, uint32_t n_reads) {
    if (n_reads && !offsets) { set_err("offsets NULL"); return TGSF_ERR_INVALID; }
    const u64 n_bases = n_reads ? offsets[n_reads] : 0;
    return submit_common(c, bases, quals, (const u64 *)offsets, n_reads, n_bases, false);
}

int tgsf_submit_packed(tgsf_ctx *c, const uint8_t *packed_bases, const uint8_t *quals, const uint64_t *offsets,
                       uint32_t n_reads, const uint64_t *exc_pos, const uint8_t *exc_byte, uint64_t n_exc) {
    if (n_reads && (!offsets || !packed_bases)) { set_err("packed/offsets NULL"); return TGSF_ERR_INVALID; }
    if (n_exc && (!exc_pos || !exc_byte)) { set_err("exception arrays NULL"); return TGSF_ERR_INVALID; }
    const u64 n_bases = n_reads ? offsets[n_reads] : 0;
    for (u64 i = 0; i < n_exc; ++i)
        if (exc_pos[i] >= n_bases) { set_err("exception position out of range"); return TGSF_ERR_INVALID; }
    PackedIn pk;
    pk.packed = packed_bases;
    pk.exc_pos = (const u64 *)exc_pos;
    pk.exc_val = exc_byte;
    pk.n_exc = n_exc;
    return submit_common(c, nullptr, quals, (const u64 *)offsets, n_reads, n_bases, false, &pk);
}

extern "C" int tgsf_pack_has_avx2();
extern "C" uint64_t tgsf_pack_groups_avx2(const uint8_t *bases, uint8_t *packed, uint64_t g0, uint64_t n_groups);

int tgsf_pack_bases(const uint8_t *bases, uint64_t n, uint8_t *packed, uint64_t *exc_pos, uint8_t *exc_byte,
                    uint64_t exc_cap, uint64_t *n_exc) {
    if ((n && (!bases || !packed)) || !n_exc) { set_err("pack: NULL argument"); return TGSF_ERR_INVALID; }
    static const struct Lut { uint8_t code[256]; Lut() { memset(code, 4, 256); code['A'] = 0; code['C'] = 1; code['G'] = 2; code['T'] = 3; } } lut;
    u64 ne = 0;
    const u64 full = n / 4;
    static const bool avx2 = tgsf_pack_has_avx2() != 0;
    const u64 groups = avx2 ? n / 32 : 0;
    auto scalar_word = [&](u64 i) {
        const uint8_t c0 = lut.code[bases[4 * i]], c1 = lut.code[bases[4 * i + 1]], c2 = lut.code[bases[4 * i + 2]],
                      c3 = lut.code[bases[4 * i + 3]];
        if ((c0 | c1 | c2 | c3) & 4) {
            uint8_t v = 0;
            for (int j = 0; j < 4; ++j) {
                const uint8_t cj = lut.code[bases[4 * i + j]];
                if (cj & 4) {
                    if (exc_pos && ne < exc_cap) { exc_pos[ne] = 4 * i + j; exc_byte[ne] = bases[4 * i + j]; }
                    ++ne;
                } else {
                    v |= (uint8_t)(cj << (2 * j));
                }
            }
            packed[i] = v;
        } else {
            packed[i] = (uint8_t)(c0 | (c1 << 2) | (c2 << 4) | (c3 << 6));
        }
    };
    u64 i = 0;
    while (i < full) {
        if ((i & 7) == 0 && (i >> 3) < groups) {
            const u64 g = tgsf_pack_groups_avx2(bases, packed, i >> 3, groups);
            i = g << 3;
            if (g < groups) {
                for (int w = 0; w < 8; ++w) scalar_word(i + (u64)w);
                i += 8;
            }
            continue;
        }
        scalar_word(i++);
    }
    if (n & 3) {
        uint8_t v = 0;
        for (u64 j = 0; j < (n & 3); ++j) {
            const uint8_t cj = lut.code[bases[4 * full + j]];
            if (cj & 4) {
                if (exc_pos && ne < exc_cap) { exc_pos[ne] = 4 * full + j; exc_byte[ne] = bases[4 * full + j]; }
                ++ne;
            } else {
                v |= (uint8_t)(cj << (2 * j));
            }
        }
        packed[full] = v;
    }
    *n_exc = ne;
    if (ne > exc_cap) { set_err("pack: %llu exceptions, capacity %llu", (unsigned long long)ne, (unsigned long long)exc_cap); return TGSF_ERR_CAPACITY; }
    return TGSF_OK;
}

int tgsf_submit_device(tgsf_ctx *c, const uint8_t *d_bases, const uint8_t *d_quals, const uint64_t *d_offsets,
                       uint32_t n_reads, uint64_t n_bases) {
    return submit_common(c, d_bases, d_quals, (const u64 *)d_offsets, n_reads, n_bases, true);
}

int tgsf_collect_gz(tgsf_ctx *c, uint8_t *blob, uint64_t blob_cap, uint64_t *blob_bytes, tgsf_gz_span *spans,
                    uint32_t spans_cap, uint32_t *n_spans) {
    if (!c || !blob_bytes || !n_spans) { set_err("collect_gz: NULL argument"); return TGSF_ERR_INVALID; }
    if (!(c->P.flags & TGSF_FLAG_GZ_BLOCKS)) { set_err("context was created without TGSF_FLAG_GZ_BLOCKS"); return TGSF_ERR_STATE; }
    if (c->outstanding == 0) { set_err("nothing outstanding"); return TGSF_ERR_STATE; }
    CU(cudaSetDevice(c->device));
    Slot &s = c->slots[c->tail];
    CU(cudaEventSynchronize(s.ev_end));
    const DevHeader *H = (const DevHeader *)s.h_header.p;
    if (H->status == DEV_STATUS_POOL_OVERFLOW) {
        set_err("collect_gz: this batch overflowed the region pool; tgsf_collect re-runs it, compress its records on the host");
        return TGSF_ERR_STATE;
    }
    if (H->gz_overflow) { set_err("deflate blob overflow"); return TGSF_ERR_CUDA; }
    const u32 np = H->tmp_cursor;
    *blob_bytes = (uint64_t)H->gz_cursor;
    *n_spans = np;
    if (H->gz_cursor > blob_cap || np > spans_cap) { set_err("collect_gz: buffers too small"); return TGSF_ERR_CAPACITY; }
    if (H->gz_cursor) CU(cudaMemcpyAsync(blob, s.gz_blob.p, (size_t)H->gz_cursor, cudaMemcpyDeviceToHost, s.stream));
    if (np) CU(cudaMemcpyAsync(spans, s.gz_spans.p, (size_t)np * sizeof(tgsf_gz_span), cudaMemcpyDeviceToHost, s.stream));
    CU(cudaStreamSynchronize(s.stream));
    return TGSF_OK;
}

int tgsf_collect(tgsf_ctx *c, tgsf_read_result *reads, uint32_t n_reads, tgsf_piece *pieces, uint32_t pieces_cap,
                 uint32_t *n_pieces) {
    if (!c) { set_err("ctx is NULL"); return TGSF_ERR_INVALID; }
    if (c->outstanding == 0) { set_err("nothing outstanding"); return TGSF_ERR_STATE; }
    CU(cudaSetDevice(c->device));
    Slot &s = c->slots[c->tail];
    CU(cudaEventSynchronize(s.ev_end));
    DevHeader *H = (DevHeader *)s.h_header.p;
    float extra_ms = 0;
    int guard = 0;
    while (H->status == DEV_STATUS_POOL_OVERFLOW && guard++ < 8) {
        u32 need = 0;
        CU(cudaMemcpy(&need, s.mid_off.as<u32>() + (size_t)s.B.n_reads * std::max(c->P.n_adapters, 1), sizeof(u32),
                      cudaMemcpyDeviceToHost));
        s.pool_cap = std::max(need + need / 4 + 1024, s.pool_cap * 2);
        TRY(slot_reserve(c, s, s.B.n_reads, s.n_bases));
        CU(cudaMemsetAsync(s.header.p, 0, sizeof(DevHeader), s.stream));
        cudaEvent_t e0, e1;
        CU(cudaEventCreate(&e0));
        CU(cudaEventCreate(&e1));
        CU(cudaEventRecord(e0, s.stream));
        TRY(launch_tail(c, s));
        CU(cudaEventRecord(e1, s.stream));
        TRY(enqueue_d2h(c, s));
        CU(cudaStreamSynchronize(s.stream));
        float ms = 0;
        cudaEventElapsedTime(&ms, e0, e1);
        extra_ms += ms;
        cudaEventDestroy(e0);
        cudaEventDestroy(e1);
    }
    float k_ms = 0, t_ms = 0;
    cudaEventElapsedTime(&k_ms, s.ev_k0, s.ev_k1);
    cudaEventElapsedTime(&t_ms, s.ev_start, s.ev_end);
    c->last_kernel_ms = k_ms + extra_ms;
    c->last_total_ms = t_ms + extra_ms;
    cudaEventElapsedTime(&c->last_span_start, c->ev_epoch, s.ev_k0);
    cudaEventElapsedTime(&c->last_span_end, c->ev_epoch, s.ev_k1);
    c->last_span_end += extra_ms;
    for (int i = 0; i < TGSF_N_STAGES; ++i) {
        float ms = 0;
        cudaEventElapsedTime(&ms, s.ev_stage[i], s.ev_stage[i + 1]);
        c->last_stage_ms[i] = ms;
    }
    c->last_chunk_shift = s.chunk_shift;

    auto retire = [&]() {
        s.busy = false;
        c->tail = (c->tail + 1) % (u32)c->slots.size();
        c->outstanding--;
    };
    if (H->status == DEV_STATUS_BIN_OVERFLOW) {
        retire();
        set_err("a read is longer than max_read_len allows (per-100 bp bins)");
        return TGSF_ERR_CAPACITY;
    }
    if (H->status != DEV_STATUS_OK) {
        retire();
        set_err("device status %u", H->status);
        return TGSF_ERR_CUDA;
    }
    const u32 total = H->tmp_cursor;
    if (n_pieces) *n_pieces = total;
    if (reads) {
        if (n_reads < s.B.n_reads) { set_err("reads array too small"); return TGSF_ERR_CAPACITY; }
        memcpy(reads, s.h_res.p, (size_t)s.B.n_reads * sizeof(tgsf_read_result));
    }
    if (pieces) {
        if (pieces_cap < total) { set_err("pieces array too small: need %u", total); return TGSF_ERR_CAPACITY; }
        const u32 have = std::min(total, s.h_pieces_copied);
        memcpy(pieces, s.h_pieces.p, (size_t)have * sizeof(tgsf_piece));
        if (total > have)
            CU(cudaMemcpy(pieces + have, s.pieces.as<tgsf_piece>() + have, (size_t)(total - have) * sizeof(tgsf_piece),
                          cudaMemcpyDeviceToHost));
    }
    retire();
    return TGSF_OK;
}

int tgsf_last_timing(tgsf_ctx *c, float *kernel_ms, float *total_ms) {
    if (!c) return TGSF_ERR_INVALID;
    if (kernel_ms) *kernel_ms = c->last_kernel_ms;
    if (total_ms) *total_ms = c->last_total_ms;
    return TGSF_OK;
}

int tgsf_last_span(tgsf_ctx *c, float *start_ms, float *end_ms) {
    if (!c) return TGSF_ERR_INVALID;
    if (start_ms) *start_ms = c->last_span_start;
    if (end_ms) *end_ms = c->last_span_end;
    return TGSF_OK;
}

int tgsf_last_stage_ms(tgsf_ctx *c, float *out, int n) {
    if (!c || !out) return TGSF_ERR_INVALID;
    for (int i = 0; i < n && i < TGSF_N_STAGES; ++i) out[i] = c->last_stage_ms[i];
    return TGSF_OK;
}

int tgsf_counter_layout_get(const tgsf_ctx *c, tgsf_counter_layout *out) {
    if (!c || !out) return TGSF_ERR_INVALID;
    *out = c->P.L;
    return TGSF_OK;
}

int tgsf_counters(tgsf_ctx *c, uint64_t *out, uint32_t n_u64) {
    if (!c || !out) return TGSF_ERR_INVALID;
    if (c->outstanding) { set_err("collect all batches first"); return TGSF_ERR_STATE; }
    if (n_u64 < c->P.L.n_u64) { set_err("counter array too small"); return TGSF_ERR_CAPACITY; }
    CU(cudaSetDevice(c->device));
    CU(cudaMemcpy(out, c->counters.p, (size_t)c->P.L.n_u64 * sizeof(u64), cudaMemcpyDeviceToHost));
    return TGSF_OK;
}

int tgsf_counters_reset(tgsf_ctx *c) {
    if (!c) return TGSF_ERR_INVALID;
    if (c->outstanding) { set_err("collect all batches first"); return TGSF_ERR_STATE; }
    CU(cudaSetDevice(c->device));
    CU(cudaMemset(c->counters.p, 0, (size_t)c->P.L.n_u64 * sizeof(u64)));
    return TGSF_OK;
}

int tgsf_counters_device(tgsf_ctx *c, void **d_ptr, uint32_t *n_u64) {
    if (!c || !d_ptr) return TGSF_ERR_INVALID;
    *d_ptr = c->counters.p;
    if (n_u64) *n_u64 = c->P.L.n_u64;
    return TGSF_OK;
}

uint64_t tgsf_launch_count(const tgsf_ctx *c) { return c ? c->launches : 0; }

int tgsf_launch_shape(const tgsf_ctx *c, int32_t *sm_count, int32_t *last_chunk_shift) {
    if (!c) { set_err("ctx is NULL"); return TGSF_ERR_INVALID; }
    if (sm_count) *sm_count = c->sm_count;
    if (last_chunk_shift) *last_chunk_shift = c->last_chunk_shift;
    return TGSF_OK;
}


int tgsf_allreduce(tgsf_ctx **ctxs, int n) {
    if (!ctxs || n <= 0) { set_err("allreduce: no contexts"); return TGSF_ERR_INVALID; }
    for (int i = 0; i < n; ++i) {
        if (!ctxs[i]) { set_err("allreduce: NULL context"); return TGSF_ERR_INVALID; }
        if (ctxs[i]->outstanding) { set_err("allreduce: collect all batches first"); return TGSF_ERR_STATE; }
        if (ctxs[i]->P.L.bc_len != ctxs[0]->P.L.bc_len) { set_err("allreduce: counter layouts differ"); return TGSF_ERR_INVALID; }
    }
    u32 bins = 0;
    for (int i = 0; i < n; ++i) bins = std::max(bins, ctxs[i]->P.L.max_bins);
    for (int i = 0; i < n; ++i)
        if (ctxs[i]->P.L.max_bins < bins) {
            CU(cudaSetDevice(ctxs[i]->device));
            TRY(grow_counters_to(ctxs[i], bins));
        }
    if (n == 1) return TGSF_OK;
    tgsf_ctx *root = ctxs[0];
    const u32 words = root->P.L.n_u64;
    const size_t bytes = (size_t)words * sizeof(u64);
    CU(cudaSetDevice(root->device));
    for (int i = 1; i < n; ++i) {
        int can = 0;
        if (cudaDeviceCanAccessPeer(&can, root->device, ctxs[i]->device) == cudaSuccess && can) {
            cudaError_t e = cudaDeviceEnablePeerAccess(ctxs[i]->device, 0);
            if (e != cudaSuccess && e != cudaErrorPeerAccessAlreadyEnabled) {  }
            cudaGetLastError();
        }
    }
    DBuf scratch;
    TRY(scratch.ensure(bytes));
    int rc = TGSF_OK;
    for (int i = 1; i < n && rc == TGSF_OK; ++i) {
        if (cudaMemcpyPeer(scratch.p, root->device, ctxs[i]->counters.p, ctxs[i]->device, bytes) != cudaSuccess) {
            set_err("allreduce: peer copy failed: %s", cudaGetErrorString(cudaGetLastError()));
            rc = TGSF_ERR_CUDA;
            break;
        }
        k_add_u64<<<root->sm_count, 256>>>(root->counters.as<u64>(), scratch.as<u64>(), words);
        root->launches++;
        if (cudaDeviceSynchronize() != cudaSuccess) { set_err("allreduce: add kernel failed"); rc = TGSF_ERR_CUDA; }
    }
    for (int i = 1; i < n && rc == TGSF_OK; ++i)
        if (cudaMemcpyPeer(ctxs[i]->counters.p, ctxs[i]->device, root->counters.p, root->device, bytes) != cudaSuccess) {
            set_err("allreduce: broadcast failed: %s", cudaGetErrorString(cudaGetLastError()));
            rc = TGSF_ERR_CUDA;
        }
    scratch.release();
    return rc;
}

int tgsf_prepass(int device, const uint8_t *ends5p, const uint8_t *ends3p, uint32_t n, uint32_t row_len,
                 const uint8_t *const *lib_seq, const int32_t *lib_len, int32_t n_lib, float min_sim,
                 int32_t *bases_num5p, int32_t *bases_num3p, int64_t *map5p, int64_t *map3p) {
    if (!ends5p || !ends3p || !bases_num5p || !bases_num3p || row_len == 0) {
        set_err("prepass: bad arguments");
        return TGSF_ERR_INVALID;
    }
    if (lib_seq && (n_lib <= 0 || n_lib > 1024 || !lib_len || !map5p || !map3p)) { set_err("prepass: bad library"); return TGSF_ERR_INVALID; }
    for (int32_t a = 0; lib_seq && a < n_lib; ++a)
        if (!lib_seq[a] || lib_len[a] <= 0 || lib_len[a] > TGSF_MAX_ADAPTER_LEN) {
            set_err("prepass: library adapter %d: length %d outside [1, %d]", a, lib_len[a], TGSF_MAX_ADAPTER_LEN);
            return TGSF_ERR_INVALID;
        }
    CU(cudaSetDevice(device));
    cudaDeviceProp prop;
    CU(cudaGetDeviceProperties(&prop, device));
    const int sms = prop.multiProcessorCount;
    DBuf d_rows, d_cnt, d_maps;
    AdapterSet ads;
    Scratch scratch;
    auto cleanup = [&]() { d_rows.release(); d_cnt.release(); d_maps.release(); ads.release(); scratch.buf.release(); };
    const size_t row_bytes = (size_t)n * row_len;
    int rc = d_rows.ensure(2 * row_bytes + 64);
    if (rc == TGSF_OK) rc = d_cnt.ensure((size_t)2 * row_len * 4 * sizeof(int));
    if (rc != TGSF_OK) { cleanup(); return rc; }
    uint8_t *r5 = d_rows.as<uint8_t>(), *r3 = r5 + row_bytes;
    cudaError_t e = cudaSuccess;
    if (row_bytes) {
        e = cudaMemcpy(r5, ends5p, row_bytes, cudaMemcpyHostToDevice);
        if (e == cudaSuccess) e = cudaMemcpy(r3, ends3p, row_bytes, cudaMemcpyHostToDevice);
    }
    if (e == cudaSuccess) e = cudaMemset(d_cnt.p, 0, (size_t)2 * row_len * 4 * sizeof(int));
    if (e != cudaSuccess) { set_err("prepass upload: %s", cudaGetErrorString(e)); cleanup(); return TGSF_ERR_CUDA; }
    int *c5 = d_cnt.as<int>(), *c3 = c5 + (size_t)row_len * 4;
    if (n) {
        const u32 tiles = cdiv(row_len, PRE_TILE_COLS);
        const dim3 grid(std::max<u32>(1, std::min<u32>(cdiv((u64)sms * 4, tiles), cdiv(n, PRE_THREADS / 32))), tiles);
        const size_t smem = (size_t)std::min<u32>(row_len, PRE_TILE_COLS) * 4 * sizeof(u32);
        k_base_content<<<grid, PRE_THREADS, smem>>>(r5, n, row_len, c5);
        k_base_content<<<grid, PRE_THREADS, smem>>>(r3, n, row_len, c3);
        rc = check_launch("k_base_content");
        if (rc != TGSF_OK) { cleanup(); return rc; }
    }
    if (lib_seq) {
        rc = ads.build(lib_seq, lib_len, n_lib);
        if (rc == TGSF_OK) {
            if (min_sim < 0.9) min_sim = 0.9;
            for (auto &A : ads.host) {
                int minK = static_cast<int>((1 - min_sim) * A.qlen) + 1;
                A.k_end = std::min(minK, A.qlen - 1);
            }
        }
        if (rc == TGSF_OK) rc = ads.upload();
        if (rc == TGSF_OK) rc = d_maps.ensure((size_t)2 * n_lib * sizeof(long long));
        if (rc == TGSF_OK) rc = scratch.ensure(ads.host, sms * 4, RES_THREADS);
        if (rc != TGSF_OK) { cleanup(); return rc; }
        e = cudaMemset(d_maps.p, 0, (size_t)2 * n_lib * sizeof(long long));
        if (e != cudaSuccess) { set_err("prepass maps: %s", cudaGetErrorString(e)); cleanup(); return TGSF_ERR_CUDA; }
        long long *m5 = d_maps.as<long long>(), *m3 = m5 + n_lib;
        const AdapterCtx AC = ads.ctx();
        for (int a = 0; a < n_lib && n; ++a) {
            const DevAdapter &Ah = ads.host[(size_t)a];
            const int grid_a = Scratch::grid_for(sms * 4, RES_THREADS, 2 * Ah.qlen + 2, Ah.nw);
            const u64 stride_a = (u64)grid_a * RES_THREADS;
            rc = for_nw(Ah.nw, [&](auto nwc) {
                constexpr int NW = decltype(nwc)::value;
                k_lib_search<NW><<<grid_a, RES_THREADS>>>(r5, n, row_len, AC, a, m5 + a, scratch.buf.as<u64>(), stride_a);
                k_lib_search<NW><<<grid_a, RES_THREADS>>>(r3, n, row_len, AC, a, m3 + a, scratch.buf.as<u64>(), stride_a);
                return check_launch("k_lib_search");
            });
            if (rc != TGSF_OK) { cleanup(); return rc; }
        }
        e = cudaMemcpy(map5p, m5, (size_t)n_lib * sizeof(long long), cudaMemcpyDeviceToHost);
        if (e == cudaSuccess) e = cudaMemcpy(map3p, m3, (size_t)n_lib * sizeof(long long), cudaMemcpyDeviceToHost);
        if (e != cudaSuccess) { set_err("prepass maps: %s", cudaGetErrorString(e)); cleanup(); return TGSF_ERR_CUDA; }
    }
    e = cudaMemcpy(bases_num5p, c5, (size_t)row_len * 4 * sizeof(int), cudaMemcpyDeviceToHost);
    if (e == cudaSuccess) e = cudaMemcpy(bases_num3p, c3, (size_t)row_len * 4 * sizeof(int), cudaMemcpyDeviceToHost);
    cleanup();
    if (e != cudaSuccess) { set_err("prepass download: %s", cudaGetErrorString(e)); return TGSF_ERR_CUDA; }
    return TGSF_OK;
}

int tgsf_align_hw(int device, const uint8_t *queries, const uint32_t *q_off, const uint8_t *targets,
                  const uint32_t *t_off, const int32_t *k, uint32_t n, tgsf_align_result *out) {
    if (!q_off || !t_off || !k || !out) { set_err("align: NULL argument"); return TGSF_ERR_INVALID; }
    if (n == 0) return TGSF_OK;
    if (n > (1u << 20)) { set_err("align: at most 2^20 pairs per call"); return TGSF_ERR_INVALID; }
    CU(cudaSetDevice(device));
    cudaDeviceProp prop;
    CU(cudaGetDeviceProperties(&prop, device));
    const int sms = prop.multiProcessorCount;
    std::vector<const uint8_t *> seqs(n);
    std::vector<int32_t> lens(n);
    for (u32 i = 0; i < n; ++i) {
        seqs[i] = queries + q_off[i];
        lens[i] = (int32_t)(q_off[i + 1] - q_off[i]);
        if (lens[i] > TGSF_MAX_ADAPTER_LEN) { set_err("align: query %u longer than %d", i, TGSF_MAX_ADAPTER_LEN); return TGSF_ERR_INVALID; }
    }
    AdapterSet ads;
    DBuf d_t, d_toff, d_k, d_out;
    Scratch scratch;
    auto cleanup = [&]() { ads.release(); d_t.release(); d_toff.release(); d_k.release(); d_out.release(); scratch.buf.release(); };
    int rc = ads.build(seqs.data(), lens.data(), (int)n);
    if (rc == TGSF_OK) {
        for (u32 i = 0; i < n; ++i)
            if (lens[i] == 0 || t_off[i + 1] == t_off[i]) ads.host[i].nw = 0;
        rc = ads.upload();
    }
    const size_t tbytes = t_off[n];
    if (rc == TGSF_OK) rc = d_t.ensure(tbytes + 64);
    if (rc == TGSF_OK) rc = d_toff.ensure(((size_t)n + 1) * sizeof(u32));
    if (rc == TGSF_OK) rc = d_k.ensure((size_t)n * sizeof(int));
    if (rc == TGSF_OK) rc = d_out.ensure((size_t)n * sizeof(tgsf_align_result));
    if (rc == TGSF_OK) rc = scratch.ensure(ads.host, sms * 2, RES_THREADS);
    if (rc != TGSF_OK) { cleanup(); return rc; }
    cudaError_t e = cudaSuccess;
    if (tbytes) e = cudaMemcpy(d_t.p, targets, tbytes, cudaMemcpyHostToDevice);
    if (e == cudaSuccess) e = cudaMemcpy(d_toff.p, t_off, ((size_t)n + 1) * sizeof(u32), cudaMemcpyHostToDevice);
    if (e == cudaSuccess) e = cudaMemcpy(d_k.p, k, (size_t)n * sizeof(int), cudaMemcpyHostToDevice);
    if (e == cudaSuccess) e = cudaMemset(d_out.p, 0, (size_t)n * sizeof(tgsf_align_result));
    if (e != cudaSuccess) { set_err("align upload: %s", cudaGetErrorString(e)); cleanup(); return TGSF_ERR_CUDA; }
    const AdapterCtx AC = ads.ctx();
    for (int nw : {1, 2, 3, 4, 8, 16, 32}) {
        int max_q = 0;
        for (u32 i = 0; i < n; ++i)
            if (ads.host[i].nw == nw) max_q = std::max(max_q, ads.host[i].qlen);
        if (max_q == 0) continue;
        const int grid_nw = Scratch::grid_for(sms * 2, RES_THREADS, 2 * max_q + 2, nw);
        rc = for_nw(nw, [&](auto nwc) {
            constexpr int NW = decltype(nwc)::value;
            k_align_pairs<NW><<<grid_nw, RES_THREADS>>>(d_t.as<uint8_t>(), d_toff.as<u32>(), d_k.as<int>(), AC, n, NW,
                                                        d_out.as<tgsf_align_result>(), scratch.buf.as<u64>(),
                                                        (u64)grid_nw * RES_THREADS);
            return check_launch("k_align_pairs");
        });
        if (rc != TGSF_OK) { cleanup(); return rc; }
    }
    e = cudaMemcpy(out, d_out.p, (size_t)n * sizeof(tgsf_align_result), cudaMemcpyDeviceToHost);
    cleanup();
    if (e != cudaSuccess) { set_err("align download: %s", cudaGetErrorString(e)); return TGSF_ERR_CUDA; }
    for (u32 i = 0; i < n; ++i) {
        if (lens[i] == 0 || t_off[i + 1] == t_off[i]) {
            tgsf_align_result R;
            memset(&R, 0, sizeof(R));
            R.edit_distance = lens[i];
            R.n_locations = 1;
            R.first_end = R.last_end = -1;
            u32 h = 2166136261u;
            const u32 v[2] = {0u, (u32)-1};
            for (int w = 0; w < 2; ++w)
                for (int b = 0; b < 4; ++b) { h ^= (v[w] >> (8 * b)) & 0xffu; h *= 16777619u; }
            R.loc_hash = h;
            out[i] = R;
        }
    }
    return TGSF_OK;
}

}
```

tgsfilter_b200/csrc/util.cuh:

```cuda
#pragma once
#include "common.cuh"

#define UTIL_THREADS 256
#define SCANB_ITEMS 8
#define SCANB_TILE (UTIL_THREADS * SCANB_ITEMS)

__global__ void __launch_bounds__(UTIL_THREADS)
k_scan_block(const u32 *__restrict__ in, u32 *__restrict__ out, u32 n, u32 *__restrict__ sums) {
    __shared__ u32 warp_tot[UTIL_THREADS / 32];
    const u32 base = blockIdx.x * SCANB_TILE + threadIdx.x * SCANB_ITEMS;
    u32 v[SCANB_ITEMS];
    u32 tsum = 0;
#pragma unroll
    for (int i = 0; i < SCANB_ITEMS; ++i) {
        v[i] = (base + i < n) ? in[base + i] : 0u;
        tsum += v[i];
    }
    const int lane = threadIdx.x & 31, warp = threadIdx.x >> 5;
    u32 inc = tsum;
#pragma unroll
    for (int o = 1; o < 32; o <<= 1) {
        const u32 t = __shfl_up_sync(0xffffffffu, inc, o);
        if (lane >= o) inc += t;
    }
    if (lane == 31) warp_tot[warp] = inc;
    __syncthreads();
    if (warp == 0) {
        u32 w = lane < UTIL_THREADS / 32 ? warp_tot[lane] : 0u;
#pragma unroll
        for (int o = 1; o < 32; o <<= 1) {
            const u32 t = __shfl_up_sync(0xffffffffu, w, o);
            if (lane >= o) w += t;
        }
        if (lane < UTIL_THREADS / 32) warp_tot[lane] = w;
    }
    __syncthreads();
    u32 excl = inc - tsum + (warp ? warp_tot[warp - 1] : 0u);
#pragma unroll
    for (int i = 0; i < SCANB_ITEMS; ++i) {
        if (base + i < n) out[base + i] = excl;
        excl += v[i];
    }
    if (threadIdx.x == UTIL_THREADS - 1) sums[blockIdx.x] = excl;
}

__global__ void __launch_bounds__(UTIL_THREADS)
k_scan_add(u32 *__restrict__ out, u32 n, const u32 *__restrict__ sums_scanned,
           const u32 *__restrict__ total) {
    const u32 i = blockIdx.x * UTIL_THREADS + threadIdx.x;
    if (i < n) out[i] += sums_scanned[i / SCANB_TILE];
    if (i == 0) out[n] = *total;
}

__global__ void k_read_segments(DevBatch B, u64 *__restrict__ seg_start, int *__restrict__ seg_len,
                                u64 *__restrict__ seg_sum, u32 *__restrict__ n_tiles, u32 max_bins,
                                u32 *__restrict__ dev_status) {
    const u32 r = blockIdx.x * blockDim.x + threadIdx.x;
    if (r >= B.n_reads) return;
    const u64 s = B.offsets[r];
    const u64 len = B.offsets[r + 1] - s;
    if (len / SCAN_BIN + 1 > (u64)max_bins || len > 0x7fffffffull) {
        *dev_status = DEV_STATUS_BIN_OVERFLOW;
        seg_len[r] = 0;
        n_tiles[r] = 0;
        seg_start[r] = s;
        seg_sum[r] = 0;
        return;
    }
    seg_start[r] = s;
    seg_len[r] = (int)len;
    seg_sum[r] = 0;
    n_tiles[r] = (u32)((len + SCAN_TILE - 1) / SCAN_TILE);
}

__global__ void k_fill_tiles(const u32 *__restrict__ tile_off, u32 n_seg,
                             const u64 *__restrict__ seg_start, const int *__restrict__ seg_len,
                             TileEntry *__restrict__ tiles) {
    const u32 s = blockIdx.x * blockDim.x + threadIdx.x;
    if (s >= n_seg) return;
    const u32 b = tile_off[s], e = tile_off[s + 1];
    const u64 s0 = seg_start[s];
    const int len = seg_len[s];
    for (u32 t = b; t < e; ++t) {
        const u32 ti = t - b;
        TileEntry te;
        te.start = s0 + (u64)ti * SCAN_TILE;
        te.seg = s;
        te.tile = (ti << TILE_N_BITS) | (u32)min(len - (int)(ti * SCAN_TILE), SCAN_TILE);
        tiles[t] = te;
    }
}

__global__ void k_count_chunks(DevBatch B, const int *__restrict__ read_active, int end_len,
                               int chunk_shift, int min_qlen, u32 *__restrict__ chunk_cnt,
                               u32 *__restrict__ best_mid, u32 *__restrict__ mid_n, int n_adapters) {
    const u32 r = blockIdx.x * blockDim.x + threadIdx.x;
    if (r >= B.n_reads) return;
    for (int a = 0; a < n_adapters; ++a) {
        best_mid[(u64)r * n_adapters + a] = 0xffffffffu;
        mid_n[(u64)r * n_adapters + a] = 0;
    }
    u32 c = 0;
    if (read_active[r]) {
        const u64 rs = B.offsets[r], re = B.offsets[r + 1];
        const i64 tsm = (i64)(re - rs) - 2 * (i64)end_len;
        if (tsm >= (i64)min_qlen && tsm > 0) {
            const u64 mb = rs + (u64)end_len, me = re - (u64)end_len;
            c = (u32)(((me - 1) >> chunk_shift) - (mb >> chunk_shift) + 1);
        }
    }
    chunk_cnt[r] = c;
}

__global__ void k_fill_chunks(DevBatch B, const u32 *__restrict__ chunk_off, int end_len,
                              int chunk_shift, ChunkEntry *__restrict__ chunks) {
    const u32 r = blockIdx.x * blockDim.x + threadIdx.x;
    if (r >= B.n_reads) return;
    const u32 b = chunk_off[r], e = chunk_off[r + 1];
    if (b == e) return;
    const u32 first = (u32)((B.offsets[r] + (u64)end_len) >> chunk_shift);
    for (u32 t = b; t < e; ++t) {
        ChunkEntry ce;
        ce.read = r;
        ce.chunk = first + (t - b);
        chunks[t] = ce;
    }
}

#define CHUNK_BUCKETS 64
static __device__ __forceinline__ u32 chunk_bucket(const DevBatch &B, u32 r, u32 chunk, int end_len,
                                                   int chunk_shift) {
    const u64 mb = B.offsets[r] + (u64)end_len, me = B.offsets[r + 1] - (u64)end_len;
    const u64 cb = (u64)chunk << chunk_shift;
    const u64 ob = max(cb, mb), oe = min(cb + (1ull << chunk_shift), me);
    const u32 len = (u32)(oe - ob);
    return (CHUNK_BUCKETS - 1) - ((len - 1) >> (chunk_shift - 6));
}

__global__ void __launch_bounds__(UTIL_THREADS)
k_chunk_hist(DevBatch B, const u32 *__restrict__ chunk_off, const ChunkEntry *__restrict__ chunks,
             int end_len, int chunk_shift, u32 *__restrict__ hist) {
    __shared__ u32 h[CHUNK_BUCKETS];
    if (threadIdx.x < CHUNK_BUCKETS) h[threadIdx.x] = 0;
    __syncthreads();
    const u32 r = blockIdx.x * UTIL_THREADS + threadIdx.x;
    if (r < B.n_reads)
        for (u32 t = chunk_off[r]; t < chunk_off[r + 1]; ++t)
            atomicAdd(&h[chunk_bucket(B, r, chunks[t].chunk, end_len, chunk_shift)], 1u);
    __syncthreads();
    if (threadIdx.x < CHUNK_BUCKETS && h[threadIdx.x]) atomicAdd(&hist[threadIdx.x], h[threadIdx.x]);
}

__global__ void k_chunk_base(u32 *__restrict__ hist) {
    if (threadIdx.x == 0) {
        u32 acc = 0;
        for (int b = 0; b < CHUNK_BUCKETS; ++b) {
            const u32 c = hist[b];
            hist[b] = acc;
            acc += c;
        }
    }
}

__global__ void __launch_bounds__(UTIL_THREADS)
k_chunk_scatter(DevBatch B, const u32 *__restrict__ chunk_off, const ChunkEntry *__restrict__ chunks,
                int end_len, int chunk_shift, u32 *__restrict__ cursor, u32 *__restrict__ perm) {
    __shared__ u32 cnt[CHUNK_BUCKETS], base[CHUNK_BUCKETS];
    if (threadIdx.x < CHUNK_BUCKETS) cnt[threadIdx.x] = 0;
    __syncthreads();
    const u32 r = blockIdx.x * UTIL_THREADS + threadIdx.x;
    const u32 b0 = r < B.n_reads ? chunk_off[r] : 0, b1 = r < B.n_reads ? chunk_off[r + 1] : 0;
    for (u32 t = b0; t < b1; ++t) atomicAdd(&cnt[chunk_bucket(B, r, chunks[t].chunk, end_len, chunk_shift)], 1u);
    __syncthreads();
    if (threadIdx.x < CHUNK_BUCKETS) {
        const u32 c = cnt[threadIdx.x];
        base[threadIdx.x] = c ? atomicAdd(&cursor[threadIdx.x], c) : 0u;
        cnt[threadIdx.x] = 0;
    }
    __syncthreads();
    for (u32 t = b0; t < b1; ++t) {
        const u32 k = chunk_bucket(B, r, chunks[t].chunk, end_len, chunk_shift);
        perm[base[k] + atomicAdd(&cnt[k], 1u)] = t;
    }
}

__global__ void k_check_pool(const u32 *__restrict__ pool_total, u32 pool_cap,
                             u32 *__restrict__ dev_status) {
    if (*pool_total > pool_cap) *dev_status = DEV_STATUS_POOL_OVERFLOW;
}

__global__ void k_add_u64(u64 *__restrict__ dst, const u64 *__restrict__ src, u32 n) {
    for (u32 i = blockIdx.x * blockDim.x + threadIdx.x; i < n; i += gridDim.x * blockDim.x) dst[i] += src[i];
}

__global__ void k_unpack_bases(const u32 *__restrict__ packed, u64 n_words, uint4 *__restrict__ out) {
    for (u64 i = (u64)blockIdx.x * blockDim.x + threadIdx.x; i < n_words; i += (u64)gridDim.x * blockDim.x) {
        const u32 w = packed[i];
        u32 o[4];
#pragma unroll
        for (int b = 0; b < 4; ++b) {
            const u32 byte = (w >> (8 * b)) & 0xffu;
            const u32 sel = (byte & 3u) | ((byte & 0xcu) << 2) | ((byte & 0x30u) << 4) | ((byte & 0xc0u) << 6);
            o[b] = __byte_perm(0x54474341u, 0u, sel);
        }
        out[i] = make_uint4(o[0], o[1], o[2], o[3]);
    }
}

__global__ void k_apply_exceptions(uint8_t *__restrict__ bases, const u64 *__restrict__ pos,
                                   const uint8_t *__restrict__ val, u64 n) {
    for (u64 i = (u64)blockIdx.x * blockDim.x + threadIdx.x; i < n; i += (u64)gridDim.x * blockDim.x)
        bases[pos[i]] = val[i];
}
```

tgsfilter_b200/engine.py:

```python
from __future__ import annotations

import ctypes as C
from typing import Optional, Tuple

import numpy as np

from . import _capi
from .params import FilterParams


class Counters:

    TABLES_BC = ("raw5p_cnt", "raw5p_qual", "raw3p_cnt", "raw3p_qual",
                 "clean5p_cnt", "clean5p_qual", "clean3p_cnt", "clean3p_qual")
    TABLES_BIN = ("raw_bin_cnt", "raw_bin_qual", "clean_bin_cnt", "clean_bin_qual")

    def __init__(self, flat: np.ndarray, layout: _capi.CounterLayout):
        self.flat = flat
        self.layout = layout
        L = layout
        self.drop_info = flat[L.drop_info:L.drop_info + _capi.DROPINFO_N]
        self.raw_hist = flat[L.raw_hist:L.raw_hist + _capi.QUAL_HIST_N]
        self.clean_hist = flat[L.clean_hist:L.clean_hist + _capi.QUAL_HIST_N]
        for name in self.TABLES_BC:
            off = getattr(L, name)
            setattr(self, name, flat[off:off + L.bc_len * 5].reshape(L.bc_len, 5))
        for name in self.TABLES_BIN:
            off = getattr(L, name)
            setattr(self, name, flat[off:off + L.max_bins * 5].reshape(L.max_bins, 5))


class FilterEngine:
    def __init__(self, params: FilterParams, device: int = 0):
        self._lib = _capi.load()
        self.params = params
        self.device = device
        p, self._keep = params.to_c()
        self._ctx = C.c_void_p()
        _capi.check(self._lib.tgsf_create(device, C.byref(p), C.byref(self._ctx)), "tgsf_create")
        self.layout = _capi.CounterLayout()
        _capi.check(self._lib.tgsf_counter_layout_get(self._ctx, C.byref(self.layout)),
                    "tgsf_counter_layout_get")
        self._inflight = []

    def close(self):
        if getattr(self, "_ctx", None) is not None and self._ctx:
            self._lib.tgsf_destroy(self._ctx)
            self._ctx = C.c_void_p()

    def __enter__(self):
        return self

    def __exit__(self, *exc):
        self.close()

    def __del__(self):
        try:
            self.close()
        except Exception:
            pass

    def set_contaminants(self, seqs, k: int = 17, min_frac: float = 0.05) -> int:
        recs = [s.encode() if isinstance(s, str) else bytes(s) for s in seqs]
        offs = np.zeros(len(recs) + 1, dtype=np.uint64)
        np.cumsum([len(r) for r in recs], out=offs[1:])
        buf = np.frombuffer(b"".join(recs) + b"\0", dtype=np.uint8)
        n = C.c_uint64(0)
        _capi.check(self._lib.tgsf_set_contaminants(self._ctx, buf.ctypes.data, offs.ctypes.data, len(recs), k,
                                                     min_frac, C.byref(n)), "tgsf_set_contaminants")
        return int(n.value)

    def submit(self, batch) -> None:
        bases = np.ascontiguousarray(batch.bases, dtype=np.uint8)
        quals = None if batch.quals is None else np.ascontiguousarray(batch.quals, dtype=np.uint8)
        offs = np.ascontiguousarray(batch.offsets, dtype=np.uint64)
        n = len(offs) - 1
        _capi.check(self._lib.tgsf_submit(
            self._ctx, bases.ctypes.data if bases.size else None,
            None if quals is None else (quals.ctypes.data if quals.size else bases.ctypes.data),
            offs.ctypes.data, n), "tgsf_submit")
        self._inflight.append((n, (bases, quals, offs)))

    def pack(self, batch):
        bases = np.ascontiguousarray(batch.bases, dtype=np.uint8)
        n = bases.size
        packed = np.zeros((n + 3) // 4 + 16, dtype=np.uint8)
        cap = 1024
        while True:
            pos = np.zeros(cap, dtype=np.uint64)
            val = np.zeros(cap, dtype=np.uint8)
            ne = C.c_uint64(0)
            rc = self._lib.tgsf_pack_bases(bases.ctypes.data if n else None, n, packed.ctypes.data,
                                           pos.ctypes.data, val.ctypes.data, cap, C.byref(ne))
            if rc == _capi.TGSF_ERR_CAPACITY:
                cap = int(ne.value)
                continue
            _capi.check(rc, "tgsf_pack_bases")
            return packed, pos[:ne.value], val[:ne.value]

    def submit_packed(self, batch, packed=None) -> None:
        if packed is None:
            packed = self.pack(batch)
        pk, pos, val = packed
        quals = None if batch.quals is None else np.ascontiguousarray(batch.quals, dtype=np.uint8)
        offs = np.ascontiguousarray(batch.offsets, dtype=np.uint64)
        n = len(offs) - 1
        _capi.check(self._lib.tgsf_submit_packed(
            self._ctx, pk.ctypes.data, None if quals is None else quals.ctypes.data, offs.ctypes.data, n,
            pos.ctypes.data if pos.size else None, val.ctypes.data if val.size else None, pos.size),
            "tgsf_submit_packed")
        self._inflight.append((n, (pk, pos, val, quals, offs)))

    def submit_packed_raw(self, packed_ptr: int, quals_ptr, offsets_ptr: int, n_reads: int,
                          exc_pos_ptr=None, exc_byte_ptr=None, n_exc: int = 0, keep=None) -> None:
        _capi.check(self._lib.tgsf_submit_packed(self._ctx, packed_ptr, quals_ptr, offsets_ptr, n_reads,
                                                 exc_pos_ptr, exc_byte_ptr, n_exc), "tgsf_submit_packed")
        self._inflight.append((n_reads, keep))

    def submit_raw(self, bases_ptr: int, quals_ptr: Optional[int], offsets_ptr: int, n_reads: int,
                   keep=None) -> None:
        _capi.check(self._lib.tgsf_submit(self._ctx, bases_ptr, quals_ptr, offsets_ptr, n_reads),
                    "tgsf_submit")
        self._inflight.append((n_reads, keep))

    def submit_device(self, d_bases: int, d_quals: Optional[int], d_offsets: int, n_reads: int,
                      n_bases: int, keep=None) -> None:
        _capi.check(self._lib.tgsf_submit_device(self._ctx, d_bases, d_quals, d_offsets, n_reads,
                                                 n_bases), "tgsf_submit_device")
        self._inflight.append((n_reads, keep))

    def collect(self, want_results: bool = True) -> Tuple[Optional[np.ndarray], Optional[np.ndarray]]:
        if not self._inflight:
            raise RuntimeError("collect() without an outstanding batch")
        n, _keep = self._inflight[0]
        npieces = C.c_uint32(0)
        if not want_results:
            rc = self._lib.tgsf_collect(self._ctx, None, 0, None, 0, C.byref(npieces))
            self._inflight.pop(0)
            _capi.check(rc, "tgsf_collect")
            return None, None
        reads = np.zeros(max(n, 1), dtype=_capi.READ_RESULT_DTYPE)
        cap = n + 4096
        pieces = np.zeros(cap, dtype=_capi.PIECE_DTYPE)
        rc = self._lib.tgsf_collect(self._ctx, reads.ctypes.data, n, pieces.ctypes.data, cap,
                                    C.byref(npieces))
        if rc == _capi.TGSF_ERR_CAPACITY and npieces.value > cap:
            cap = npieces.value
            pieces = np.zeros(cap, dtype=_capi.PIECE_DTYPE)
            rc = self._lib.tgsf_collect(self._ctx, reads.ctypes.data, n, pieces.ctypes.data, cap,
                                        C.byref(npieces))
        self._inflight.pop(0)
        _capi.check(rc, "tgsf_collect")
        return reads[:n], pieces[:npieces.value]

    def collect_gz(self):
        if not self._inflight:
            raise RuntimeError("collect_gz() without an outstanding batch")
        n, _keep = self._inflight[0]
        span_dtype = np.dtype([("offset", "<u8"), ("bytes", "<u4"), ("reserved", "<u4")])
        blob = np.zeros(1 << 20, dtype=np.uint8)
        spans = np.zeros(n + 4096, dtype=span_dtype)
        nb, ns = C.c_uint64(0), C.c_uint32(0)
        rc = self._lib.tgsf_collect_gz(self._ctx, blob.ctypes.data, blob.size, C.byref(nb), spans.ctypes.data,
                                       spans.size, C.byref(ns))
        if rc == _capi.TGSF_ERR_CAPACITY:
            blob = np.zeros(max(int(nb.value), 1), dtype=np.uint8)
            spans = np.zeros(max(int(ns.value), 1), dtype=span_dtype)
            rc = self._lib.tgsf_collect_gz(self._ctx, blob.ctypes.data, blob.size, C.byref(nb), spans.ctypes.data,
                                           spans.size, C.byref(ns))
        _capi.check(rc, "tgsf_collect_gz")
        return blob[:nb.value], spans[:ns.value]

    def run(self, batch):
        self.submit(batch)
        return self.collect()

    def last_timing(self) -> Tuple[float, float]:
        k, t = C.c_float(0), C.c_float(0)
        _capi.check(self._lib.tgsf_last_timing(self._ctx, C.byref(k), C.byref(t)), "tgsf_last_timing")
        return k.value, t.value

    def last_span(self) -> Tuple[float, float]:
        a, b = C.c_float(0), C.c_float(0)
        _capi.check(self._lib.tgsf_last_span(self._ctx, C.byref(a), C.byref(b)), "tgsf_last_span")
        return a.value, b.value

    def last_stage_ms(self) -> dict:
        arr = (C.c_float * _capi.N_STAGES)()
        _capi.check(self._lib.tgsf_last_stage_ms(self._ctx, arr, _capi.N_STAGES), "tgsf_last_stage_ms")
        return dict(zip(_capi.STAGE_NAMES, [float(x) for x in arr]))

    def counters(self) -> Counters:
        _capi.check(self._lib.tgsf_counter_layout_get(self._ctx, C.byref(self.layout)), "tgsf_counter_layout_get")
        flat = np.zeros(self.layout.n_u64, dtype=np.uint64)
        _capi.check(self._lib.tgsf_counters(self._ctx, flat.ctypes.data, flat.size), "tgsf_counters")
        return Counters(flat, self.layout)

    def reset_counters(self) -> None:
        _capi.check(self._lib.tgsf_counters_reset(self._ctx), "tgsf_counters_reset")

    def counters_device_ptr(self) -> Tuple[int, int]:
        p, n = C.c_void_p(), C.c_uint32(0)
        _capi.check(self._lib.tgsf_counters_device(self._ctx, C.byref(p), C.byref(n)),
                    "tgsf_counters_device")
        return p.value, n.value

    def launch_count(self) -> int:
        return int(self._lib.tgsf_launch_count(self._ctx))

    def launch_shape(self) -> Tuple[int, int]:
        sm, shift = C.c_int32(0), C.c_int32(0)
        _capi.check(self._lib.tgsf_launch_shape(self._ctx, C.byref(sm), C.byref(shift)), "tgsf_launch_shape")
        return sm.value, shift.value


def align_hw(pairs, device: int = 0) -> np.ndarray:
    lib = _capi.load()
    n = len(pairs)
    q_off = np.zeros(n + 1, dtype=np.uint32)
    t_off = np.zeros(n + 1, dtype=np.uint32)
    np.cumsum([len(p[0]) for p in pairs], out=q_off[1:])
    np.cumsum([len(p[1]) for p in pairs], out=t_off[1:])
    q = np.frombuffer(b"".join(p[0] for p in pairs) + b"\0", dtype=np.uint8).copy()
    t = np.frombuffer(b"".join(p[1] for p in pairs) + b"\0", dtype=np.uint8).copy()
    k = np.array([p[2] for p in pairs], dtype=np.int32)
    out = np.zeros(n, dtype=_capi.ALIGN_RESULT_DTYPE)
    _capi.check(lib.tgsf_align_hw(device, q.ctypes.data, q_off.ctypes.data, t.ctypes.data,
                                  t_off.ctypes.data, k.ctypes.data, n, out.ctypes.data),
                "tgsf_align_hw")
    return out
```

Measured before the change: 335.4.

## Scan runs of consecutive chunks per thread in mid-adapter Myers kernel

The mid-scan kernel now assigns each thread a run of several consecutive chunks, so the halo only has to be replayed once per run instead of once per chunk. The best-score tracking is rewritten as a precomputed threshold comparison, and peq row addressing uses a multiply-high trick with vectorised 16-byte shared loads. The cost is longer per-thread work items, which can worsen load balance, plus extra run-count and scheduling kernels.

```diff
diff --git a/include/tgsf.h b/include/tgsf.h
--- a/include/tgsf.h
+++ b/include/tgsf.h
@@ -157,6 +157,7 @@
 int tgsf_allreduce(tgsf_ctx **ctxs, int n);
 uint64_t tgsf_launch_count(const tgsf_ctx *ctx);
 int tgsf_launch_shape(const tgsf_ctx *ctx, int32_t *sm_count, int32_t *last_chunk_shift);
+int tgsf_mid_run_shift(const tgsf_ctx *ctx, int32_t *last_run_shift);
 
 int tgsf_prepass(int device, const uint8_t *ends5p, const uint8_t *ends3p, uint32_t n,
                  uint32_t row_len, const uint8_t *const *lib_seq, const int32_t *lib_len,
diff --git a/profiles/sass_mix.py b/profiles/sass_mix.py
--- /dev/null
+++ b/profiles/sass_mix.py
@@ -0,0 +1,133 @@
+#!/usr/bin/env python3
+from __future__ import annotations
+
+import argparse
+import collections
+import os
+import re
+import subprocess
+import sys
+import tempfile
+
+ROOT = os.path.dirname(os.path.dirname(os.path.abspath(__file__)))
+SRC = os.path.join(ROOT, "tgsfilter_b200", "csrc", "tgsf_cuda.cu")
+
+PIPES = [
+    ("alu", {"LOP3", "LOP", "IADD3", "IADD", "VIADD", "SHF", "SHL", "SHR", "ISETP", "SEL", "LEA", "PLOP3", "IMNMX", "VIMNMX",
+             "VIMNMX3", "VIADDMNMX", "PRMT", "BMSK", "SGXT", "P2R", "R2P", "IABS", "FSEL", "FSETP", "FMNMX"}),
+    ("fma", {"IMAD", "IMUL", "FFMA", "FMUL", "FADD", "HFMA2"}),
+    ("popc/flo", {"POPC", "FLO", "BREV"}),
+    ("lsu", {"LDS", "LDG", "STS", "STG", "LD", "ST", "LDL", "STL", "ATOM", "ATOMS", "ATOMG", "RED", "LDC"}),
+    ("uniform", {"S2UR", "R2UR", "ULDC"}),
+    ("control", {"BRA", "BSSY", "BSYNC", "CALL", "RET", "EXIT", "WARPSYNC", "NOP", "BAR", "YIELD", "BREAK"}),
+]
+
+LINE = re.compile(r"^\s*/\*([0-9a-f]{4,})\*/\s+(?:@!?U?P[0-9T]\s+)?([A-Z0-9_]+)((?:\.[A-Z0-9_]+)*)\s*(.*?);")
+
+
+def pipe_of(op: str) -> str:
+    for name, ops in PIPES:
+        if op in ops:
+            return name
+    if op.startswith("U"):
+        return "uniform"
+    return "other"
+
+
+def compile_cubin(out_dir: str) -> tuple[str, str]:
+    cubin = os.path.join(out_dir, "tgsf_cuda.cubin")
+    nvcc = os.environ.get("NVCC", "nvcc")
+    cmd = [nvcc, "-gencode", "arch=compute_100a,code=sm_100a", "-O3", "-std=c++17", "-cubin", "-Xptxas", "-v",
+           "-o", cubin, SRC]
+    r = subprocess.run(cmd, check=True, capture_output=True, text=True, cwd=ROOT)
+    return cubin, r.stdout + r.stderr
+
+
+def function_sass(cubin: str, mangled_prefix: str) -> tuple[str, list[tuple[int, str, str, str]]]:
+    sass = subprocess.run(["cuobjdump", "-sass", cubin], check=True, capture_output=True, text=True).stdout
+    name, body = None, []
+    for line in sass.splitlines():
+        if "Function :" in line:
+            if name is not None:
+                break
+            fn = line.split("Function :", 1)[1].strip()
+            if fn.startswith(mangled_prefix):
+                name = fn
+            continue
+        if name is not None:
+            m = LINE.match(line)
+            if m:
+                body.append((int(m.group(1), 16), m.group(2), m.group(3), m.group(4)))
+    if name is None:
+        sys.exit(f"no function {mangled_prefix}* in {cubin}")
+    return name, body
+
+
+def loops_with_wide_loads(body):
+    loops = []
+    for addr, op, mods, args in body:
+        if op == "BRA":
+            m = re.search(r"0x([0-9a-f]+)", args)
+            if m and int(m.group(1), 16) <= addr:
+                loops.append((int(m.group(1), 16), addr))
+    inner = [lp for lp in loops if not any(o != lp and lp[0] <= o[0] and o[1] <= lp[1] for o in loops)]
+    return [lp for lp in inner
+            if any(lp[0] <= a <= lp[1] and op == "LDG" and ".128" in mods for a, op, mods, _ in body)]
+
+
+def ptxas_resources(log: str, name: str) -> str:
+    lines = log.splitlines()
+    for i, line in enumerate(lines):
+        if "Compiling entry function" in line and f"'{name}'" in line:
+            out = []
+            for l in lines[i + 1:i + 6]:
+                if "Compiling entry function" in l:
+                    break
+                if "stack frame" in l or "Used" in l:
+                    out.append(l.split("info    :")[-1].strip())
+            return "; ".join(out)
+    return "not found in the ptxas log"
+
+
+def main():
+    ap = argparse.ArgumentParser(description=__doc__.split("\n\n")[0])
+    ap.add_argument("--nw", type=int, default=1, help="Myers words per adapter (template NW)")
+    ap.add_argument("--ap", type=int, default=2, help="adapters per thread (template AP)")
+    ap.add_argument("--cubin", help="use this cubin instead of compiling")
+    ap.add_argument("--ptxas-log", help="with --cubin: the -Xptxas -v output of that compile")
+    args = ap.parse_args()
+
+    with tempfile.TemporaryDirectory(prefix="sass_mix_") as tmp:
+        if args.cubin:
+            cubin = args.cubin
+            log = open(args.ptxas_log).read() if args.ptxas_log else ""
+        else:
+            cubin, log = compile_cubin(tmp)
+        name, body = function_sass(cubin, f"_Z14k_mid_scan_dynILi{args.nw}ELi{args.ap}E")
+
+    cols = 16 * args.ap
+    print(f"k_mid_scan_dyn<{args.nw},{args.ap}>  ({name})")
+    if log:
+        print(f"  ptxas: {ptxas_resources(log, name)}")
+    loops = sorted(loops_with_wide_loads(body), key=lambda lp: lp[1] - lp[0])
+    if not loops:
+        sys.exit("no loop with a 16-byte load found")
+    for i, (lo, hi) in enumerate(loops):
+        label = "hot loop (tracked columns)" if i == len(loops) - 1 else "halo loop"
+        ins = [(op, mods) for a, op, mods, _ in body if lo <= a <= hi]
+        by_op = collections.Counter(op + (".X" if op in ("IADD3", "IMAD") and ".X" in mods else "")
+                                    + (".MOV" if op == "IMAD" and ".MOV" in mods else "")
+                                    + (".SHL" if op == "IMAD" and ".SHL" in mods else "")
+                                    + (".HI" if op == "IMAD" and ".HI" in mods else "") for op, mods in ins)
+        by_pipe = collections.Counter()
+        for op, _ in ins:
+            by_pipe[pipe_of(op)] += 1
+        print(f"\n  {label}: 0x{lo:x}..0x{hi:x}, {len(ins)} instructions = {len(ins) / cols:.2f} per adapter-column "
+              f"({cols} adapter-columns per iteration)")
+        for pipe, n in sorted(by_pipe.items(), key=lambda kv: -kv[1]):
+            print(f"    {pipe:10s} {n:5d}  {n / cols:6.2f} per adapter-column")
+        print("    by opcode: " + ", ".join(f"{op} {n / cols:.2f}" for op, n in by_op.most_common()))
+
+
+if __name__ == "__main__":
+    main()
diff --git a/tgsfilter_b200/_capi.py b/tgsfilter_b200/_capi.py
--- a/tgsfilter_b200/_capi.py
+++ b/tgsfilter_b200/_capi.py
@@ -106,7 +106,7 @@
     "tgsf_version", "tgsf_last_error", "tgsf_create", "tgsf_destroy", "tgsf_device_count", "tgsf_host_alloc",
     "tgsf_host_free", "tgsf_submit", "tgsf_submit_packed", "tgsf_pack_bases", "tgsf_submit_device", "tgsf_collect", "tgsf_collect_gz", "tgsf_last_timing", "tgsf_last_span", "tgsf_last_stage_ms",
     "tgsf_counter_layout_get", "tgsf_counters", "tgsf_counters_reset", "tgsf_counters_device",
-    "tgsf_launch_count", "tgsf_launch_shape", "tgsf_allreduce", "tgsf_prepass", "tgsf_align_hw", "tgsf_set_contaminants",
+    "tgsf_launch_count", "tgsf_launch_shape", "tgsf_mid_run_shift", "tgsf_allreduce", "tgsf_prepass", "tgsf_align_hw", "tgsf_set_contaminants",
 )
 
 _lib = None
@@ -147,6 +147,7 @@
     lib.tgsf_launch_count.restype = C.c_uint64
     lib.tgsf_launch_count.argtypes = [vp]
     lib.tgsf_launch_shape.argtypes = [vp, C.POINTER(C.c_int32), C.POINTER(C.c_int32)]
+    lib.tgsf_mid_run_shift.argtypes = [vp, C.POINTER(C.c_int32)]
     lib.tgsf_allreduce.argtypes = [C.POINTER(vp), C.c_int]
     lib.tgsf_prepass.argtypes = [C.c_int, u8p, u8p, C.c_uint32, C.c_uint32,
                                  C.POINTER(C.c_char_p), C.POINTER(C.c_int32), C.c_int32, C.c_float,
diff --git a/tgsfilter_b200/csrc/adapters.cuh b/tgsfilter_b200/csrc/adapters.cuh
--- a/tgsfilter_b200/csrc/adapters.cuh
+++ b/tgsfilter_b200/csrc/adapters.cuh
@@ -24,8 +24,10 @@
     int a[2];
     int end_len;
     int chunk_shift;
+    int run_shift;
     u32 chunk_stride;
     int n_adapters;
+    u32 byte_mul[4];
 };
 
 template <int NW>
@@ -47,7 +49,8 @@
 
 template <int NW>
 static __device__ __noinline__ int mid_replay_group(const u64 *P0, const u64 *M0, u32 w0, u32 w1,
-                                                    const u64 *tab, int tab_stride, int best) {
+                                                    const u64 *tab, int tab_stride, int thr) {
+    int best = 0x7fffffff;
     u64 tP[NW], tM[NW];
 #pragma unroll
     for (int w = 0; w < NW; ++w) { tP[w] = P0[w]; tM[w] = M0[w]; }
@@ -58,17 +61,23 @@
         myers_step_state<NW>(tP, tM, tab + byte * tab_stride);
         best = min(best, myers_score<NW>(tP, tM));
     }
-    return best;
+    return min(thr, 2 * best + 6);
+}
+
+static __device__ __forceinline__ u32 mid_row_off(const u32 (&wd)[4], int j, const u32 (&mul)[4]) {
+    const u32 w = wd[j >> 2];
+    const u32 top = (j & 3) == 3 ? w : w * mul[j & 3];
+    return __umulhi(top, mul[2]) * mul[3];
 }
 
 template <int NW, int AP>
 __global__ void __launch_bounds__(MID_THREADS, (NW * AP <= 2) ? 6 : 3)
-k_mid_scan_dyn(DevBatch B, AdapterCtx C, MidScanArgs M, const ChunkEntry *__restrict__ chunks,
-               const u32 *__restrict__ perm, const u32 *__restrict__ n_chunks_ptr,
-               uint8_t *__restrict__ chunk_min,
+k_mid_scan_dyn(DevBatch B, AdapterCtx C, MidScanArgs M, const u32 *__restrict__ chunk_off,
+               const ChunkEntry *__restrict__ runs, const u32 *__restrict__ perm,
+               const u32 *__restrict__ n_runs_ptr, uint8_t *__restrict__ chunk_min,
                u32 *__restrict__ chunk_cnt, u64 *__restrict__ chunk_first,
                u32 *__restrict__ best_mid, u32 *__restrict__ work_ctr) {
-    const u32 n_chunks = *n_chunks_ptr;
+    const u32 n_runs = *n_runs_ptr;
     extern __shared__ __align__(16) u64 s_peq_smem[];
     DevAdapter A[AP];
 #pragma unroll
@@ -86,7 +95,8 @@
         __syncthreads();
     }
     constexpr int TS = AP * NW;
-    const u64 chunk_len = 1ull << M.chunk_shift;
+    const int cs = M.chunk_shift;
+    const u64 chunk_len = 1ull << cs;
     int halo = 0, qmin = 0x7fffffff;
 #pragma unroll
     for (int x = 0; x < AP; ++x) {
@@ -94,28 +104,29 @@
         qmin = min(qmin, A[x].qlen);
     }
     const uint4 *__restrict__ b16 = (const uint4 *)B.bases;
+    int thr0[AP];
+#pragma unroll
+    for (int x = 0; x < AP; ++x) thr0[x] = 2 * A[x].k_mid + 8;
 
     const u32 lane = threadIdx.x & 31u;
     for (;;) {
         u32 it = 0;
         if (lane == 0) it = atomicAdd(work_ctr, 32u);
         it = __shfl_sync(0xffffffffu, it, 0);
-        if (it >= n_chunks) break;
+        if (it >= n_runs) break;
         it += lane;
-        if (it >= n_chunks) continue;
-        const u32 ci = perm[it];
-        const ChunkEntry ce = chunks[ci];
-        const u64 rs = B.offsets[ce.read];
-        const u64 re = B.offsets[ce.read + 1];
-        const i64 tsm = (i64)(re - rs) - 2 * (i64)M.end_len;
-        const u64 mb = rs + (u64)M.end_len, me = re - (u64)M.end_len;
-        const u64 cb = (u64)ce.chunk << M.chunk_shift;
-        const u64 ob = max(cb, mb), oe = min(cb + chunk_len, me);
-        u64 sb = ob > (u64)halo ? ob - (u64)halo : 0;
-        if (sb < mb) sb = mb;
+        if (it >= n_runs) continue;
+        const ChunkEntry re = runs[perm[it]];
+        const u64 rs = B.offsets[re.read];
+        const i64 tsm = (i64)(B.offsets[re.read + 1] - rs) - 2 * (i64)M.end_len;
+        const u64 mb = rs + (u64)M.end_len, me = B.offsets[re.read + 1] - (u64)M.end_len;
+        const u32 c_first = (u32)(mb >> cs);
+        u32 c = max(re.chunk << M.run_shift, c_first);
+        const u32 c_last = min(((re.chunk + 1) << M.run_shift) - 1u, (u32)((me - 1) >> cs));
+        u32 ci = chunk_off[re.read] + (c - c_first);
 
         u64 Pv[AP][NW], Mv[AP][NW];
-        int score[AP], best[AP];
+        int score[AP], thr[AP];
         bool on[AP];
 #pragma unroll
         for (int x = 0; x < AP; ++x) {
@@ -124,79 +135,116 @@
 #pragma unroll
             for (int w = 0; w < NW; ++w) { Pv[x][w] = s0.Pv[w]; Mv[x][w] = s0.Mv[w]; }
             score[x] = A[x].qlen;
-            best[x] = 0x7fffffff;
+            thr[x] = thr0[x];
             on[x] = A[x].k_mid > 0 && tsm >= (i64)A[x].qlen;
         }
-        if (tsm >= (i64)qmin) {
-            u64 p = sb;
-            while (p < oe && (p & 15ull)) {
+        const bool scan = tsm >= (i64)qmin;
+        u64 ob = max((u64)c << cs, mb);
+        u64 sb = ob > (u64)halo ? ob - (u64)halo : 0;
+        if (sb < mb) sb = mb;
+        u64 p = sb;
+        if (scan) {
+            const u64 oe0 = min(((u64)c << cs) + chunk_len, me);
+            while (p < oe0 && (p & 15ull)) {
                 const u64 *eq = s_peq + (u32)B.bases[p] * TS;
 #pragma unroll
                 for (int x = 0; x < AP; ++x) {
                     myers_step_state<NW>(Pv[x], Mv[x], eq + x * NW);
                     score[x] = myers_score<NW>(Pv[x], Mv[x]);
-                    if (p >= ob) best[x] = min(best[x], score[x]);
+                    if (p >= ob) thr[x] = min(thr[x], 2 * score[x] + 6);
                 }
                 ++p;
             }
-            for (; p + 16 <= oe; p += 16) {
+            for (; p < ob; p += 16) {
                 const uint4 v = __ldg(b16 + (p >> 4));
                 const u32 wd[4] = {v.x, v.y, v.z, v.w};
-                const bool tracked = p >= ob;
-#pragma unroll
-                for (int h = 0; h < 2; ++h) {
-                    u64 Pv0[AP][NW], Mv0[AP][NW];
-#pragma unroll
-                    for (int x = 0; x < AP; ++x)
-#pragma unroll
-                        for (int w = 0; w < NW; ++w) { Pv0[x][w] = Pv[x][w]; Mv0[x][w] = Mv[x][w]; }
-#pragma unroll
-                    for (int j = 8 * h; j < 8 * h + 8; ++j) {
-                        const u32 byte = (wd[j >> 2] >> (8 * (j & 3))) & 0xffu;
-                        const u64 *eq = s_peq + byte * TS;
-#pragma unroll
-                        for (int x = 0; x < AP; ++x) myers_step_state<NW>(Pv[x], Mv[x], eq + x * NW);
-                    }
-                    if (tracked) {
+#pragma unroll
+                for (int j = 0; j < 16; ++j) {
+                    const u64 *eq = s_peq + ((wd[j >> 2] >> (8 * (j & 3))) & 0xffu) * TS;
+#pragma unroll
+                    for (int x = 0; x < AP; ++x) myers_step_state<NW>(Pv[x], Mv[x], eq + x * NW);
+                }
+            }
+#pragma unroll
+            for (int x = 0; x < AP; ++x) score[x] = myers_score<NW>(Pv[x], Mv[x]);
+        }
+        for (;;) {
+            const u64 cb = (u64)c << cs;
+            const u64 oe = min(cb + chunk_len, me);
+            if (scan && p < oe) {
+                const uint4 *q = b16 + (p >> 4);
+                for (u32 g = (u32)((oe - p) >> 4); g; --g, ++q) {
+                    const uint4 v = __ldg(q);
+                    const u32 wd[4] = {v.x, v.y, v.z, v.w};
+#pragma unroll
+                    for (int h = 0; h < 2; ++h) {
+                        u64 Pv0[AP][NW], Mv0[AP][NW];
+#pragma unroll
+                        for (int x = 0; x < AP; ++x)
+#pragma unroll
+                            for (int w = 0; w < NW; ++w) { Pv0[x][w] = Pv[x][w]; Mv0[x][w] = Mv[x][w]; }
+#pragma unroll
+                        for (int j = 8 * h; j < 8 * h + 8; ++j) {
+                            const char *row = (const char *)s_peq + mid_row_off(wd, j, M.byte_mul);
+                            u64 eq[TS];
+                            if constexpr (TS % 2 == 0) {
+#pragma unroll
+                                for (int i = 0; i < TS; i += 2) {
+                                    const ulonglong2 v = *(const ulonglong2 *)(row + 8 * i);
+                                    eq[i] = v.x;
+                                    eq[i + 1] = v.y;
+                                }
+                            } else {
+#pragma unroll
+                                for (int i = 0; i < TS; ++i) eq[i] = *(const u64 *)(row + 8 * i);
+                            }
+#pragma unroll
+                            for (int x = 0; x < AP; ++x) myers_step_state<NW>(Pv[x], Mv[x], eq + x * NW);
+                        }
 #pragma unroll
                         for (int x = 0; x < AP; ++x) {
                             const int s_end = myers_score<NW>(Pv[x], Mv[x]);
-                            if (((score[x] + s_end - 8 + 1) >> 1) <= min(A[x].k_mid, best[x] - 1))
-                                best[x] = mid_replay_group<NW>(Pv0[x], Mv0[x], wd[2 * h], wd[2 * h + 1],
-                                                               s_peq + x * NW, TS, best[x]);
+                            if (score[x] + s_end <= thr[x])
+                                thr[x] = mid_replay_group<NW>(Pv0[x], Mv0[x], wd[2 * h], wd[2 * h + 1],
+                                                              s_peq + x * NW, TS, thr[x]);
                             score[x] = s_end;
                         }
                     }
                 }
-                if (!tracked && p + 16 >= ob) {
-#pragma unroll
-                    for (int x = 0; x < AP; ++x) score[x] = myers_score<NW>(Pv[x], Mv[x]);
-                }
-            }
-            for (; p < oe; ++p) {
-                const u64 *eq = s_peq + (u32)B.bases[p] * TS;
-#pragma unroll
-                for (int x = 0; x < AP; ++x) {
-                    myers_step_state<NW>(Pv[x], Mv[x], eq + x * NW);
-                    score[x] = myers_score<NW>(Pv[x], Mv[x]);
-                    if (p >= ob) best[x] = min(best[x], score[x]);
-                }
-            }
-        }
-#pragma unroll
-        for (int x = 0; x < AP; ++x) {
-            uint8_t result = 255;
-            const u64 slot = (u64)M.a[x] * M.chunk_stride + ci;
-            if (on[x] && best[x] <= A[x].k_mid) {
-                result = (uint8_t)min(best[x], 254);
-                atomicMin(best_mid + (u64)ce.read * M.n_adapters + M.a[x], (u32)best[x]);
-                u32 cnt;
-                u64 first;
-                mid_chunk_record<NW>(s_peq + x * NW, TS, A[x].qlen, B.bases, sb, ob, oe, best[x], cnt, first);
-                chunk_cnt[slot] = cnt;
-                chunk_first[slot] = first | ((u64)best[x] << 48);
-            }
-            chunk_min[slot] = result;
+                p = oe & ~15ull;
+                for (; p < oe; ++p) {
+                    const u64 *eq = s_peq + (u32)B.bases[p] * TS;
+#pragma unroll
+                    for (int x = 0; x < AP; ++x) {
+                        myers_step_state<NW>(Pv[x], Mv[x], eq + x * NW);
+                        score[x] = myers_score<NW>(Pv[x], Mv[x]);
+                        thr[x] = min(thr[x], 2 * score[x] + 6);
+                    }
+                }
+            }
+#pragma unroll
+            for (int x = 0; x < AP; ++x) {
+                uint8_t result = 255;
+                const u64 slot = (u64)M.a[x] * M.chunk_stride + ci;
+                if (on[x] && thr[x] < thr0[x]) {
+                    const int best = (thr[x] - 6) >> 1;
+                    result = (uint8_t)min(best, 254);
+                    atomicMin(best_mid + (u64)re.read * M.n_adapters + M.a[x], (u32)best);
+                    const u64 cob = max(cb, mb);
+                    u64 csb = cob > (u64)halo ? cob - (u64)halo : 0;
+                    if (csb < mb) csb = mb;
+                    u32 cnt;
+                    u64 first;
+                    mid_chunk_record<NW>(s_peq + x * NW, TS, A[x].qlen, B.bases, csb, cob, oe, best, cnt, first);
+                    chunk_cnt[slot] = cnt;
+                    chunk_first[slot] = first | ((u64)best << 48);
+                }
+                chunk_min[slot] = result;
+                thr[x] = thr0[x];
+            }
+            if (c == c_last) break;
+            ++c;
+            ++ci;
         }
     }
 }
diff --git a/tgsfilter_b200/csrc/common.cuh b/tgsfilter_b200/csrc/common.cuh
--- a/tgsfilter_b200/csrc/common.cuh
+++ b/tgsfilter_b200/csrc/common.cuh
@@ -16,6 +16,7 @@
 #define SCAN_TILE (SCAN_BIN * SCAN_TILE_BINS)
 #define MID_CHUNK_SHIFT_MIN 10
 #define MID_CHUNK_SHIFT_MAX 12
+#define MID_RUN_BLOCK_SHIFT 12
 
 struct DevAdapter {
     int qlen;
diff --git a/tgsfilter_b200/csrc/tgsf_cuda.cu b/tgsfilter_b200/csrc/tgsf_cuda.cu
--- a/tgsfilter_b200/csrc/tgsf_cuda.cu
+++ b/tgsfilter_b200/csrc/tgsf_cuda.cu
@@ -208,13 +208,14 @@
     u64 n_bases = 0;
     bool has_qual = false;
     DBuf seg_start, seg_len, seg_sum, seg_flag, tile_cnt, tile_off, tiles;
-    DBuf read_active, piece_cnt, piece_begin, chunk_cnt, chunk_off, chunks, chunk_min, chunk_hits, chunk_first, chunk_perm, chunk_hist;
-    int chunk_shift = MID_CHUNK_SHIFT_MIN;
+    DBuf read_active, piece_cnt, piece_begin, chunk_cnt, chunk_off, chunks, chunk_min, chunk_hits, chunk_first;
+    DBuf run_cnt, run_off, runs, run_perm, run_hist;
+    int chunk_shift = MID_CHUNK_SHIFT_MIN, run_shift = 0;
     DBuf best_mid, mid_n, mid_off, end_n, end_pos, pool, sortbuf, tmp, pieces, res, header;
     DBuf scan_tmp, kmer_long_list, mid_work, gz_blob, gz_spans;
     DBuf contam_cnt, contam_off, contam_chunks;
     Scratch scratch, scratch2;
-    u32 pool_cap = 0, pieces_cap = 0, chunks_cap = 0, tiles_cap = 0;
+    u32 pool_cap = 0, pieces_cap = 0, chunks_cap = 0, runs_cap = 0, tiles_cap = 0;
     HBuf h_res, h_pieces, h_header;
     u32 h_pieces_copied = 0;
     float kernel_ms = 0, total_ms = 0;
@@ -250,6 +251,7 @@
     float last_kernel_ms = 0, last_total_ms = 0;
     float last_stage_ms[TGSF_N_STAGES] = {};
     int last_chunk_shift = 0;
+    int last_run_shift = 0;
     cudaEvent_t ev_epoch = nullptr;
     float last_span_start = 0, last_span_end = 0;
 };
@@ -296,7 +298,8 @@
 void slot_release(Slot &s) {
     DBuf *bufs[] = {&s.in_bases, &s.in_quals, &s.in_offsets, &s.in_packed, &s.in_exc_pos, &s.in_exc_val, &s.seg_start, &s.seg_len, &s.seg_sum,
                     &s.seg_flag, &s.tile_cnt, &s.tile_off, &s.tiles, &s.read_active, &s.piece_cnt,
-                    &s.piece_begin, &s.chunk_cnt, &s.chunk_off, &s.chunks, &s.chunk_min, &s.chunk_hits, &s.chunk_first, &s.chunk_perm, &s.chunk_hist,
+                    &s.piece_begin, &s.chunk_cnt, &s.chunk_off, &s.chunks, &s.chunk_min, &s.chunk_hits, &s.chunk_first,
+                    &s.run_cnt, &s.run_off, &s.runs, &s.run_perm, &s.run_hist,
                     &s.best_mid, &s.mid_n, &s.mid_off, &s.end_n, &s.end_pos, &s.pool, &s.sortbuf,
                     &s.tmp, &s.pieces, &s.res, &s.header, &s.scan_tmp, &s.kmer_long_list, &s.mid_work, &s.gz_blob, &s.gz_spans, &s.scratch.buf, &s.scratch2.buf,
                     &s.contam_cnt, &s.contam_off, &s.contam_chunks};
@@ -325,6 +328,8 @@
            (n_bases >> (s.chunk_shift + 1)) >= (u64)c->sm_count * 2048ull * 4ull)
         s.chunk_shift++;
     s.chunks_cap = (u32)((n_bases >> s.chunk_shift) + 2ull * n + 16);
+    s.run_shift = MID_RUN_BLOCK_SHIFT - s.chunk_shift;
+    s.runs_cap = (u32)((n_bases >> (s.chunk_shift + s.run_shift)) + 2ull * n + 16);
     s.tiles_cap = (u32)(n_bases / SCAN_TILE + (u64)s.pieces_cap + 16);
     const size_t nseg = std::max<size_t>(n, s.pieces_cap) + 1;
     TRY(s.seg_start.ensure(nseg * sizeof(u64)));
@@ -343,8 +348,11 @@
     TRY(s.chunk_min.ensure((size_t)s.chunks_cap * (size_t)A));
     TRY(s.chunk_hits.ensure((size_t)s.chunks_cap * (size_t)A * sizeof(u32)));
     TRY(s.chunk_first.ensure((size_t)s.chunks_cap * (size_t)A * sizeof(u64)));
-    TRY(s.chunk_perm.ensure((size_t)s.chunks_cap * sizeof(u32)));
-    TRY(s.chunk_hist.ensure(CHUNK_BUCKETS * sizeof(u32)));
+    TRY(s.run_cnt.ensure(((size_t)n + 1) * sizeof(u32)));
+    TRY(s.run_off.ensure(((size_t)n + 2) * sizeof(u32)));
+    TRY(s.runs.ensure((size_t)s.runs_cap * sizeof(ChunkEntry)));
+    TRY(s.run_perm.ensure((size_t)s.runs_cap * sizeof(u32)));
+    TRY(s.run_hist.ensure(CHUNK_BUCKETS * sizeof(u32)));
     TRY(s.best_mid.ensure(((size_t)n * A + 1) * sizeof(u32)));
     TRY(s.mid_n.ensure(((size_t)n * A + 1) * sizeof(u32)));
     TRY(s.mid_off.ensure(((size_t)n * A + 2) * sizeof(u32)));
@@ -517,24 +525,28 @@
             TRY(launch_ends(s.stream2, s.scratch2));
             CU(cudaEventRecord(s.ev_join, s.stream2));
         }
-        k_count_chunks<<<cdiv(n, 256), 256, 0, st>>>(s.B, s.read_active.as<int>(), P.end_len, s.chunk_shift, c->ads.min_q,
-                                                     s.chunk_cnt.as<u32>(), s.best_mid.as<u32>(),
-                                                     s.mid_n.as<u32>(), A);
+        k_count_chunks<<<cdiv(n, 256), 256, 0, st>>>(s.B, s.read_active.as<int>(), P.end_len, s.chunk_shift, s.run_shift,
+                                                     c->ads.min_q, s.chunk_cnt.as<u32>(), s.run_cnt.as<u32>(),
+                                                     s.best_mid.as<u32>(), s.mid_n.as<u32>(), A);
         c->launches++;
         TRY(exclusive_scan(c, st, s.chunk_cnt.as<u32>(), s.chunk_off.as<u32>(), n, s.scan_tmp.as<u32>(),
                            s.scan_tmp.cap / sizeof(u32)));
+        TRY(exclusive_scan(c, st, s.run_cnt.as<u32>(), s.run_off.as<u32>(), n, s.scan_tmp.as<u32>(),
+                           s.scan_tmp.cap / sizeof(u32)));
+        const int run_block = s.chunk_shift + s.run_shift;
         k_fill_chunks<<<cdiv(n, 256), 256, 0, st>>>(s.B, s.chunk_off.as<u32>(), P.end_len, s.chunk_shift, s.chunks.as<ChunkEntry>());
-        c->launches++;
-        CU(cudaMemsetAsync(s.chunk_hist.p, 0, CHUNK_BUCKETS * sizeof(u32), st));
-        k_chunk_hist<<<cdiv(n, UTIL_THREADS), UTIL_THREADS, 0, st>>>(s.B, s.chunk_off.as<u32>(), s.chunks.as<ChunkEntry>(),
-                                                                   P.end_len, s.chunk_shift, s.chunk_hist.as<u32>());
-        k_chunk_base<<<1, 32, 0, st>>>(s.chunk_hist.as<u32>());
-        k_chunk_scatter<<<cdiv(n, UTIL_THREADS), UTIL_THREADS, 0, st>>>(s.B, s.chunk_off.as<u32>(), s.chunks.as<ChunkEntry>(),
-                                                                      P.end_len, s.chunk_shift, s.chunk_hist.as<u32>(),
-                                                                      s.chunk_perm.as<u32>());
+        k_fill_chunks<<<cdiv(n, 256), 256, 0, st>>>(s.B, s.run_off.as<u32>(), P.end_len, run_block, s.runs.as<ChunkEntry>());
+        c->launches += 2;
+        CU(cudaMemsetAsync(s.run_hist.p, 0, CHUNK_BUCKETS * sizeof(u32), st));
+        k_chunk_hist<<<cdiv(n, UTIL_THREADS), UTIL_THREADS, 0, st>>>(s.B, s.run_off.as<u32>(), s.runs.as<ChunkEntry>(),
+                                                                   P.end_len, run_block, s.run_hist.as<u32>());
+        k_chunk_base<<<1, 32, 0, st>>>(s.run_hist.as<u32>());
+        k_chunk_scatter<<<cdiv(n, UTIL_THREADS), UTIL_THREADS, 0, st>>>(s.B, s.run_off.as<u32>(), s.runs.as<ChunkEntry>(),
+                                                                      P.end_len, run_block, s.run_hist.as<u32>(),
+                                                                      s.run_perm.as<u32>());
         c->launches += 3;
         const AdapterCtx AC = c->ads.ctx();
-        const u32 *n_chunks_ptr = s.chunk_off.as<u32>() + n;
+        const u32 *n_runs_ptr = s.run_off.as<u32>() + n;
         const int res_grid = c->sm_count * c->res_ctas_per_sm;
         int mid_launch = 0;
         CU(cudaMemsetAsync(s.mid_work.p, 0, (size_t)A * sizeof(u32), st));
@@ -550,24 +562,29 @@
                 M.a[1] = pair ? grp[i + 1] : grp[i];
                 M.end_len = P.end_len;
                 M.chunk_shift = s.chunk_shift;
+                M.run_shift = s.run_shift;
                 M.chunk_stride = s.chunks_cap;
                 M.n_adapters = A;
+                M.byte_mul[0] = 1u << 24;
+                M.byte_mul[1] = 1u << 16;
+                M.byte_mul[2] = 1u << 8;
                 TRY(for_nw(nw, [&](auto nwc) {
                     constexpr int NW = decltype(nwc)::value;
-                    auto launch = [&](auto kern, size_t smem) {
+                    auto launch = [&](auto kern, size_t smem, int ap) {
+                        M.byte_mul[3] = (u32)(8 * ap * NW);
                         int occ = 0;
                         if (cudaOccupancyMaxActiveBlocksPerMultiprocessor(&occ, kern, MID_THREADS, smem) != cudaSuccess || occ < 1) occ = 4;
                         if (c->mid_ctas_per_sm > 0) occ = std::min(occ, c->mid_ctas_per_sm);
                         kern<<<c->sm_count * occ, MID_THREADS, smem, st>>>(
-                            s.B, AC, M, s.chunks.as<ChunkEntry>(), s.chunk_perm.as<u32>(), n_chunks_ptr,
+                            s.B, AC, M, s.chunk_off.as<u32>(), s.runs.as<ChunkEntry>(), s.run_perm.as<u32>(), n_runs_ptr,
                             s.chunk_min.as<uint8_t>(), s.chunk_hits.as<u32>(), s.chunk_first.as<u64>(),
                             s.best_mid.as<u32>(), s.mid_work.as<u32>() + mid_launch);
                     };
                     if constexpr (NW <= 4) {
-                        if (pair) launch(k_mid_scan_dyn<NW, 2>, 256 * 2 * NW * sizeof(u64));
-                        else launch(k_mid_scan_dyn<NW, 1>, 256 * NW * sizeof(u64));
+                        if (pair) launch(k_mid_scan_dyn<NW, 2>, 256 * 2 * NW * sizeof(u64), 2);
+                        else launch(k_mid_scan_dyn<NW, 1>, 256 * NW * sizeof(u64), 1);
                     } else {
-                        launch(k_mid_scan_dyn<NW, 1>, 0);
+                        launch(k_mid_scan_dyn<NW, 1>, 0, 1);
                     }
                     c->launches++;
                     ++mid_launch;
@@ -1247,6 +1264,7 @@
         c->last_stage_ms[i] = ms;
     }
     c->last_chunk_shift = s.chunk_shift;
+    c->last_run_shift = s.run_shift;
 
     auto retire = [&]() {
         s.busy = false;
@@ -1337,6 +1355,12 @@
     if (!c) { set_err("ctx is NULL"); return TGSF_ERR_INVALID; }
     if (sm_count) *sm_count = c->sm_count;
     if (last_chunk_shift) *last_chunk_shift = c->last_chunk_shift;
+    return TGSF_OK;
+}
+
+int tgsf_mid_run_shift(const tgsf_ctx *c, int32_t *last_run_shift) {
+    if (!c) { set_err("ctx is NULL"); return TGSF_ERR_INVALID; }
+    if (last_run_shift) *last_run_shift = c->last_run_shift;
     return TGSF_OK;
 }
 
diff --git a/tgsfilter_b200/csrc/util.cuh b/tgsfilter_b200/csrc/util.cuh
--- a/tgsfilter_b200/csrc/util.cuh
+++ b/tgsfilter_b200/csrc/util.cuh
@@ -92,33 +92,36 @@
 }
 
 __global__ void k_count_chunks(DevBatch B, const int *__restrict__ read_active, int end_len,
-                               int chunk_shift, int min_qlen, u32 *__restrict__ chunk_cnt,
-                               u32 *__restrict__ best_mid, u32 *__restrict__ mid_n, int n_adapters) {
+                               int chunk_shift, int run_shift, int min_qlen, u32 *__restrict__ chunk_cnt,
+                               u32 *__restrict__ run_cnt, u32 *__restrict__ best_mid, u32 *__restrict__ mid_n,
+                               int n_adapters) {
     const u32 r = blockIdx.x * blockDim.x + threadIdx.x;
     if (r >= B.n_reads) return;
     for (int a = 0; a < n_adapters; ++a) {
         best_mid[(u64)r * n_adapters + a] = 0xffffffffu;
         mid_n[(u64)r * n_adapters + a] = 0;
     }
-    u32 c = 0;
+    u32 c = 0, n = 0;
     if (read_active[r]) {
         const u64 rs = B.offsets[r], re = B.offsets[r + 1];
         const i64 tsm = (i64)(re - rs) - 2 * (i64)end_len;
         if (tsm >= (i64)min_qlen && tsm > 0) {
             const u64 mb = rs + (u64)end_len, me = re - (u64)end_len;
             c = (u32)(((me - 1) >> chunk_shift) - (mb >> chunk_shift) + 1);
+            n = (u32)(((me - 1) >> (chunk_shift + run_shift)) - (mb >> (chunk_shift + run_shift)) + 1);
         }
     }
     chunk_cnt[r] = c;
+    run_cnt[r] = n;
 }
 
 __global__ void k_fill_chunks(DevBatch B, const u32 *__restrict__ chunk_off, int end_len,
-                              int chunk_shift, ChunkEntry *__restrict__ chunks) {
+                              int block_shift, ChunkEntry *__restrict__ chunks) {
     const u32 r = blockIdx.x * blockDim.x + threadIdx.x;
     if (r >= B.n_reads) return;
     const u32 b = chunk_off[r], e = chunk_off[r + 1];
     if (b == e) return;
-    const u32 first = (u32)((B.offsets[r] + (u64)end_len) >> chunk_shift);
+    const u32 first = (u32)((B.offsets[r] + (u64)end_len) >> block_shift);
     for (u32 t = b; t < e; ++t) {
         ChunkEntry ce;
         ce.read = r;
@@ -129,24 +132,24 @@
 
 #define CHUNK_BUCKETS 64
 static __device__ __forceinline__ u32 chunk_bucket(const DevBatch &B, u32 r, u32 chunk, int end_len,
-                                                   int chunk_shift) {
+                                                   int block_shift) {
     const u64 mb = B.offsets[r] + (u64)end_len, me = B.offsets[r + 1] - (u64)end_len;
-    const u64 cb = (u64)chunk << chunk_shift;
-    const u64 ob = max(cb, mb), oe = min(cb + (1ull << chunk_shift), me);
+    const u64 cb = (u64)chunk << block_shift;
+    const u64 ob = max(cb, mb), oe = min(cb + (1ull << block_shift), me);
     const u32 len = (u32)(oe - ob);
-    return (CHUNK_BUCKETS - 1) - ((len - 1) >> (chunk_shift - 6));
+    return (CHUNK_BUCKETS - 1) - ((len - 1) >> (block_shift - 6));
 }
 
 __global__ void __launch_bounds__(UTIL_THREADS)
 k_chunk_hist(DevBatch B, const u32 *__restrict__ chunk_off, const ChunkEntry *__restrict__ chunks,
-             int end_len, int chunk_shift, u32 *__restrict__ hist) {
+             int end_len, int block_shift, u32 *__restrict__ hist) {
     __shared__ u32 h[CHUNK_BUCKETS];
     if (threadIdx.x < CHUNK_BUCKETS) h[threadIdx.x] = 0;
     __syncthreads();
     const u32 r = blockIdx.x * UTIL_THREADS + threadIdx.x;
     if (r < B.n_reads)
         for (u32 t = chunk_off[r]; t < chunk_off[r + 1]; ++t)
-            atomicAdd(&h[chunk_bucket(B, r, chunks[t].chunk, end_len, chunk_shift)], 1u);
+            atomicAdd(&h[chunk_bucket(B, r, chunks[t].chunk, end_len, block_shift)], 1u);
     __syncthreads();
     if (threadIdx.x < CHUNK_BUCKETS && h[threadIdx.x]) atomicAdd(&hist[threadIdx.x], h[threadIdx.x]);
 }
@@ -164,13 +167,13 @@
 
 __global__ void __launch_bounds__(UTIL_THREADS)
 k_chunk_scatter(DevBatch B, const u32 *__restrict__ chunk_off, const ChunkEntry *__restrict__ chunks,
-                int end_len, int chunk_shift, u32 *__restrict__ cursor, u32 *__restrict__ perm) {
+                int end_len, int block_shift, u32 *__restrict__ cursor, u32 *__restrict__ perm) {
     __shared__ u32 cnt[CHUNK_BUCKETS], base[CHUNK_BUCKETS];
     if (threadIdx.x < CHUNK_BUCKETS) cnt[threadIdx.x] = 0;
     __syncthreads();
     const u32 r = blockIdx.x * UTIL_THREADS + threadIdx.x;
     const u32 b0 = r < B.n_reads ? chunk_off[r] : 0, b1 = r < B.n_reads ? chunk_off[r + 1] : 0;
-    for (u32 t = b0; t < b1; ++t) atomicAdd(&cnt[chunk_bucket(B, r, chunks[t].chunk, end_len, chunk_shift)], 1u);
+    for (u32 t = b0; t < b1; ++t) atomicAdd(&cnt[chunk_bucket(B, r, chunks[t].chunk, end_len, block_shift)], 1u);
     __syncthreads();
     if (threadIdx.x < CHUNK_BUCKETS) {
         const u32 c = cnt[threadIdx.x];
@@ -179,7 +182,7 @@
     }
     __syncthreads();
     for (u32 t = b0; t < b1; ++t) {
-        const u32 k = chunk_bucket(B, r, chunks[t].chunk, end_len, chunk_shift);
+        const u32 k = chunk_bucket(B, r, chunks[t].chunk, end_len, block_shift);
         perm[base[k] + atomicAdd(&cnt[k], 1u)] = t;
     }
 }
diff --git a/tgsfilter_b200/engine.py b/tgsfilter_b200/engine.py
--- a/tgsfilter_b200/engine.py
+++ b/tgsfilter_b200/engine.py
@@ -213,6 +213,11 @@
         _capi.check(self._lib.tgsf_launch_shape(self._ctx, C.byref(sm), C.byref(shift)), "tgsf_launch_shape")
         return sm.value, shift.value
 
+    def mid_run_shift(self) -> int:
+        rs = C.c_int32(0)
+        _capi.check(self._lib.tgsf_mid_run_shift(self._ctx, C.byref(rs)), "tgsf_mid_run_shift")
+        return rs.value
+
 
 def align_hw(pairs, device: int = 0) -> np.ndarray:
     lib = _capi.load()
```

Measured after the change: 350.6 (median of 6 runs). 1.05x the previous value.
